# xxayt/MGSV

Measured on AMD Instinct MI355X. Metric: video-music pairs/s fwd+bwd at B=64 (full training step); sub-objects: retrieval sim-matrix GB/s, eval forward pairs/s, higher is better.
Workload: dtype bf16; 1 GPU; BASELINE.json configs[2]: B=64/GPU, T_v=30, T_a=512, D=512, train mode (dropout on), f32 master weights + Adam, f32 gradient accumulation; global_batch=64, launch=tape

## Files before the change

include/made_hip.h:

```cpp
#ifndef MADE_HIP_H
#define MADE_HIP_H

#include <stdint.h>

#ifdef __cplusplus
extern "C" {
#endif

#define MADE_ABI_VERSION 8

enum MadeDtype { MADE_F32 = 0, MADE_BF16 = 1 };

enum MadeAct {
    MADE_ACT_NONE = 0,
    MADE_ACT_RELU = 1,
    MADE_ACT_GELU = 2,
    MADE_ACT_QUICKGELU = 3,
    MADE_ACT_SIGMOID = 4
};

enum MadeGate {
    MADE_GATE_NONE = 0,
    MADE_GATE_RELU_OUT = 1,
    MADE_GATE_GELU_Z = 2,
// ... 20 lines not shown
MADE_HOST_DEVICE static inline uint32_t made_drop_threshold(float p) { return (uint32_t)((double)p * 16777216.0); }
MADE_HOST_DEVICE static inline uint32_t made_rng_key(uint64_t seed, uint32_t site, uint32_t idx_hi) {
    return made_rng_fmix32((uint32_t)seed ^ (site * 0x9E3779B9u) ^ ((uint32_t)(seed >> 32) * 0x85EBCA6Bu) ^ (idx_hi * 0xC2B2AE35u));
}
MADE_HOST_DEVICE static inline uint32_t made_rng_mix(uint64_t seed, uint32_t site, uint64_t idx) {
    return made_rng_fmix32((uint32_t)idx ^ made_rng_key(seed, site, (uint32_t)(idx >> 32)));
}
#if defined(__HIPCC__)
__device__ static inline uint64_t made_drop_seed(const MadeDropout& d) { return d.seed_device ? *d.seed_device : d.seed; }
#endif


enum MadeStatus {
    MADE_OK = 0,
    MADE_ERR_INVALID_ARG = -1,
    MADE_ERR_UNSUPPORTED = -2,
    MADE_ERR_HIP = -3
};

int         made_abi_version(void);
int         made_set_f32_products(int mode);
int         made_get_f32_products(void);
const char* made_last_error(void);
int         made_device_info(char* name, int name_len, int* cu_count, int* is_gfx950);

typedef struct MadeLinearSeg {
    int64_t col_begin;
    void*   out;
    int32_t out_dtype;
    int32_t transposed;
    int64_t ldo;
    int64_t rows_per_batch;
    int64_t out_batch_stride;
    int64_t out_z_stride;
    int32_t use_a2;
    int32_t _pad;
} MadeLinearSeg;

typedef struct MadeLinearArgs {
    const void*  A;  int32_t a_dtype; int32_t w_dtype;
    int64_t      lda;
    const void*  A2; int64_t lda2; int64_t a2_row_mod;
    int32_t      a2_replace;
    int32_t      drop_col_div;
    const float* a_row_mask;
    const void*  W;  int64_t ldw;
    const float* bias;
    int64_t      M, N, K;
    int64_t      batch, a_z_stride, w_z_stride;
    int32_t      act; int32_t r_dtype;
    const void*  R;  int64_t ldr; int64_t r_row_mod;
    const float* out_row_mask;
    const float* tile_skip_mask;
    int32_t      nseg; int32_t split_k;
    float*       split_ws;
    MadeLinearSeg seg[4];
    const void*  G;  int32_t g_dtype; int32_t gate;
    int64_t      ldg; float gate_scale; int32_t z_dtype;
    void*        Zout; int64_t ldz;
    MadeDropout  drop; int64_t drop_ld;
    const int32_t* row_index; const int32_t* n_rows;
    const float* bias_row_scale; int64_t bias_z_stride;
} MadeLinearArgs;

int made_linear(const MadeLinearArgs* args, void* stream);

enum MadeLinearVariant {
    MADE_LINEAR_GENERAL_F32 = 0,
    MADE_LINEAR_GENERAL_F32IN = 1,
    MADE_LINEAR_GENERAL_BF16 = 2,
    MADE_LINEAR_TINY = 3,
    MADE_LINEAR_SKINNY = 4,
    MADE_LINEAR_GLDS3 = 5,
    MADE_LINEAR_GLDS64 = 6,
    MADE_LINEAR_GLDS128 = 7,
    MADE_LINEAR_BIG256 = 8,
    MADE_LINEAR_TINY16 = 9,
    MADE_LINEAR_BIG128 = 10,
    MADE_LINEAR_GLDS64_F32 = 11,
    MADE_LINEAR_GLDS128_F32 = 12
};
int made_linear_variant(const MadeLinearArgs* args);

typedef struct MadeDecStageArgs {
    const void*  Zin; int64_t ldz;
    const float* ln_g; const float* ln_b;
    const float* ln2_g; const float* ln2_b; void* x2_out; int64_t ldx2;
    const void*  add; int64_t add_row_mod;
    void*        x_out; int64_t ldx;
    const void*  W; int64_t ldw; const float* bias;
    const void*  R; int64_t ldr;
    void*        out; int64_t ldo;
    int32_t      out_dtype; int32_t act; int32_t res_from_x; float eps;
    int64_t      M, N, K;
    int32_t      zin_dtype; int32_t drop_col_div;
    void*        a_out; int64_t lda_out;
    MadeDropout  drop; int64_t drop_ld;
} MadeDecStageArgs;
int made_dec_stage(const MadeDecStageArgs* args, void* stream);

typedef struct MadeDecStageBwdArgs {
    const void* xa; const float* gamma_a; int64_t ldxa;
    const void* xb; const float* gamma_b; int64_t ldxb;
    const void* dy; int64_t lddy;
    const void* add; int64_t ldadd;
    void* dx_out; int64_t lddx;
    void* a_out; int64_t lda_out;
    float *dgamma_a, *dbeta_a, *dgamma_b, *dbeta_b;
    MadeDropout drop_a; int64_t drop_a_ld;
    const void* W; int64_t ldw;
    const void* G; int64_t ldg; float gate_scale; float eps;
    MadeDropout drop_o; int64_t drop_o_ld; int32_t drop_o_col_div; int32_t _pad;
    const void* R; int64_t ldr;
    void* out; int64_t ldo;
    int64_t M, N, K;
} MadeDecStageBwdArgs;
int made_dec_stage_bwd(const MadeDecStageBwdArgs* args, void* stream);

typedef struct MadeFinishArgs {
    const float* ws; int64_t split_k, M, N;
    const float* bias; int32_t act; int32_t r_dtype;
    const void*  R; int64_t ldr; int64_t r_row_mod;
    void* out; int32_t out_dtype; int32_t _pad0; int64_t ldo;
    const float* ln1_g; const float* ln1_b; void* ln1_out; int32_t ln1_dtype; int32_t _pad1; int64_t ln1_ld;
    const float* ln2_g; const float* ln2_b; void* ln2_out; int32_t ln2_dtype; int32_t _pad2; int64_t ln2_ld;
    float eps; int32_t _pad3;
} MadeFinishArgs;

int made_splitk_finish(const MadeFinishArgs* args, void* stream);

typedef struct MadeAttnArgs {
    const void* Q; const void* K; const void* V; void* O;
    int32_t dtype; int32_t hd;
    int64_t B, H, Lq, Lk;
    int64_t q_bs, ldq, k_bs, ldk, v_bs, ldv, o_bs, ldo;
    const float* key_mask; const float* q_mask;
    float scale; int32_t _pad;
    const float* q_skip_mask;
    float*      lse;
    MadeDropout drop;
    const int32_t* batch_order;
    uint32_t* keep_bits;
    int64_t ld_bits;
} MadeAttnArgs;

int made_attention(const MadeAttnArgs* args, void* stream);

typedef struct MadeWideAttnArgs {
    const void* Q; const void* K; const void* Kadd; const void* V; void* O;
    const float* key_mask;
    int32_t dtype; int32_t o_dtype;
    int64_t B, NQ1, NQ2, L, D;
    int64_t q_bs, q_s1, q_s2, k_bs, ldk, kadd_bs, ldkadd, v_bs, ldv, o_bs, o_s1, o_s2;
    float scale; int32_t _pad;
    int64_t n_split;
    float*  part_o;
    float*  part_ml;
    MadeDropout drop;
    float*  sum_out;
    float*  lse_out;
} MadeWideAttnArgs;

int made_attention_wide(const MadeWideAttnArgs* args, void* stream);

typedef struct MadeWideAttnBwdArgs {
    const void *Q, *dO, *O, *K, *V;
// ... 219 lines not shown
typedef struct MadeGemmTNGroup {
    int32_t n_problems; float alpha;
    int64_t M, split_m;
    const int32_t* row_index; const int32_t* n_rows;
    MadeGemmTNProblem p[MADE_GEMM_TN_MAX_GROUP];
    int32_t tile_end[MADE_GEMM_TN_MAX_GROUP];
    int32_t tile_size; int32_t _pad;
    void* workspace; int64_t workspace_bytes;
} MadeGemmTNGroup;
int made_gemm_tn_grouped(const MadeGemmTNGroup* group, void* stream);
int64_t made_gemm_tn_grouped_workspace(const MadeGemmTNGroup* group);
int made_row_groups(const float* mask, int64_t M, float* out, void* stream);
int made_row_index(const float* mask, int64_t M, int32_t* row_index, int32_t* n_rows, void* stream);
int made_batch_order(const float* mask, int64_t B, int64_t T, int32_t* order, void* stream);

int made_layernorm_bwd(const void* x, int32_t x_dtype, int64_t ldx, int64_t x_rows_per_batch, int64_t x_batch_stride,
                       const float* gamma, const void* dy, int32_t dy_dtype, int64_t lddy,
                       const void* add, int32_t add_dtype, int64_t ld_add,
                       void* dx, int32_t dx_dtype, int64_t lddx,
                       void* dx_drop, int64_t lddxd, const MadeDropout* drop, int64_t drop_ld,
                       float* dgamma, float* dbeta, int64_t rows, int64_t D, float eps, const float* row_skip, void* stream);

int made_pool_bwd(const float* mean, const float* dvec, const float* mask,
                  const void* in1, int32_t in1_dtype, int64_t in1_bs, int64_t in1_ld,
                  const void* in2, int32_t in2_dtype, int64_t in2_bs, int64_t in2_ld,
                  void* out, int32_t out_dtype, int64_t out_bs, int64_t out_ld,
                  int64_t B, int64_t T, int64_t D, float eps, void* stream);

int made_l2norm_bwd(const void* x, int32_t x_dtype, int64_t ldx, const float* dy, int64_t lddy, int64_t dy_rows_per,
                    float* dx, int64_t lddx, int32_t accumulate, void* dx_alt, int32_t alt_dtype, int64_t lddxa,
                    int64_t rows, int64_t D, float eps, void* stream);

int made_clip_loss_bwd(const float* sims, int64_t ld, int64_t n, const float* logit_scale, float weight,
                       const float* upstream, float* lse_ws, float* dsims, float* dsims_t, int32_t accumulate,
                       float* d_logit_scale, const float* row_exclude, void* stream);

int made_xpool_tail_bwd(const void* y, int32_t y_dtype, int64_t ldy, const float* gamma, const float* beta,
                        const float* video, int64_t ld_video, const float* dsims, int64_t ld_dsims,
                        void* dy, int32_t dy_dtype, int64_t lddy, void* dy_drop, const MadeDropout* drop,
                        float* dgamma, float* dbeta, float* dvideo, int64_t ld_dvideo,
                        const float* dpool, int64_t ld_dpool, float dpool_scale,
                        int64_t Nm, int64_t Nv, int64_t D, float eps, void* stream);

int made_softmax_bwd(const float* S, int64_t ld_s, const float* dP, int64_t ld_dp, const float* mask, int64_t rows_per_mask,
                     const float* extra, float scale, const MadeDropout* drop,
                     void* Pd, void* dS, void* dSt, int32_t out_dtype, int64_t ldo, int64_t ldt,
                     int64_t out_batch_stride, int64_t t_batch_stride,
                     int64_t rows, int64_t rows_per_batch, int64_t L, void* stream);

int made_head_bias(void* x, int32_t x_dtype, int64_t ldx, const float* s, const float* bias, int64_t rows, int64_t H, int64_t hd,
                   void* stream);
int made_head_bias_bwd(const void* dy, int32_t dtype, int64_t ld, const float* s, const float* bias, float* dbias, float* ds,
                       int64_t rows, int64_t H, int64_t hd, void* stream);

int made_layernorm_bwd2(const void* xa, const float* gamma_a, int64_t ldxa, const void* xb, const float* gamma_b, int64_t ldxb,
                        const void* dy, int64_t lddy, const void* add, int64_t ld_add, void* dx, int64_t lddx,
                        void* dx_drop, int64_t lddxd, const MadeDropout* drop, int64_t drop_ld, int32_t dtype,
                        float* dgamma_a, float* dbeta_a, float* dgamma_b, float* dbeta_b, int64_t rows, int64_t D, float eps,
                        void* stream);

int made_gate_rows(const void* x, int32_t x_dtype, int64_t ldx, const void* G, int32_t g_dtype, int64_t ldg, int32_t gate,
                   float scale, const MadeDropout* drop, int64_t drop_ld, int64_t drop_col_div, void* out, int32_t out_dtype, int64_t ldo,
                   const float* row_skip, int64_t rows, int64_t cols, void* stream);
int made_add3(void* out, int32_t out_dtype, const void* a, int32_t a_dtype, const void* b, int32_t b_dtype,
              const void* c, int32_t c_dtype, int64_t n, int64_t b_mod, void* stream);
int made_colsum(const void* x, int32_t dtype, int64_t ld, int64_t rows, int64_t cols, float* out, void* stream);

int made_posbn_relu_fwd(const void* x, int32_t x_dtype, int64_t ldx, const float* weight, const float* bias,
                        float* running_mean, float* running_var, float momentum, float eps, int32_t batch_stats,
                        float* save_mean, float* save_rstd, void* y, int32_t y_dtype, int64_t ldy,
                        int64_t B, int64_t T, int64_t F, void* stream);
int made_posbn_relu_bwd(const void* x, int32_t x_dtype, int64_t ldx, const void* y, int32_t y_dtype, int64_t ldy,
                        const void* dy, int32_t dy_dtype, int64_t lddy, const float* weight, const float* save_mean,
                        const float* save_rstd, int32_t batch_stats, void* dx, int32_t dx_dtype, int64_t lddx,
                        float* dweight, float* dbias, int64_t B, int64_t T, int64_t F, void* stream);

int made_set_criterion_bwd(const float* pred_logits, const float* pred_spans, const float* targets,
                           const int64_t* pred_idx, const int64_t* tgt_idx, const int32_t* count,
                           const float* proj_queries, const float* vid_sum, const float* empty_weight,
                           int64_t n_layers, int64_t B, int64_t Q, int64_t G, int64_t Dc, int32_t fg_label,
                           float temperature, const float* weights, const float* upstream,
                           float* d_logits, float* d_spans, int64_t ld_out, int32_t through_sigmoid,
                           float* d_proj_queries, float* d_vid_sum, void* stream);

#define MADE_ADAM_MAX_GROUPS 4
#define MADE_ADAM_NORM_BLOCKS 1024
typedef struct MadeAdamGroup { int64_t begin, end; float lr; float max_norm; } MadeAdamGroup;
int made_adam_step(float* param, const float* grad, float* exp_avg, float* exp_avg_sq, int64_t n,
                   const MadeAdamGroup* groups, int32_t n_groups, float beta1, float beta2, float eps, int64_t step,
                   float grad_scale, float* norm_ws, void* stream);

typedef struct MadeAdamDeviceState { int64_t step; float lr[MADE_ADAM_MAX_GROUPS]; float bc1, bc2_sqrt; } MadeAdamDeviceState;
int made_adam_step_device(float* param, const float* grad, float* exp_avg, float* exp_avg_sq, int64_t n,
                          const MadeAdamGroup* groups, int32_t n_groups, float beta1, float beta2, float eps,
                          MadeAdamDeviceState* state_device, int32_t advance_state, float grad_scale, float* norm_ws, void* stream);

typedef struct MadeRepackDesc {
    const float* src; void* w; void* wt;
    int64_t rows, cols, wt_ld, tile_begin;
    int32_t dtype; int32_t _pad;
} MadeRepackDesc;
int made_repack(const MadeRepackDesc* descs_device, int32_t n_desc, int64_t total_tiles, void* stream);


int made_recall_ranks(const float* sims, int64_t ld, const int32_t* group_id, const int32_t* gt_group, int64_t Nv, int64_t Nm,
                      int64_t n_groups, int32_t* rank_out, int32_t* top1_out, void* stream);

int made_span_iou(const float* pred_logits, const float* pred_spans, const float* gt_moment, const float* m_duration,
                  int64_t N, int64_t Q, int32_t fg_label, float max_m_duration, float* iou_out, float* pred_out, void* stream);

int made_concat_cols(const float* a, int64_t cols_a, const float* c, int64_t cols_c, float* out, int64_t rows, void* stream);


int made_pooled_cosine(const float* anchor, int64_t lda, const void* pooled, int32_t pooled_dtype, float* out, int64_t sa, int64_t sp,
                       int64_t A, int64_t P, int64_t D, void* stream);
int made_scale_exp(const float* x, const float* logit_scale, float* out, int64_t n, void* stream);
int made_span_convert(const float* in, float* out, int64_t N, int32_t mode, void* stream);
int made_span_pairwise(const float* spans1, const float* spans2, float* iou, float* uni, float* giou, float* inter_over_2,
                       int64_t N, int64_t M, void* stream);
int made_span_iou_se(const float* pred_se, const float* gt_moment, const float* m_duration, int64_t N, float max_m_duration,
                     int32_t clamp_to_max, int32_t discounted, float* iou_out, void* stream);


int64_t made_topk_groups_ws_bytes(int64_t Nv, int64_t Nm, int64_t K);
int made_topk_groups(const float* sims, int64_t ld, const int32_t* group_id, int64_t Nv, int64_t Nm, int64_t n_groups,
                     int64_t K, int32_t* idx_out, float* score_out, void* ws, int64_t ws_bytes, void* stream);

int made_gather_pairs(const int32_t* vi, const int32_t* mi, int64_t P, int64_t Nv, int64_t Nm,
                      const void* v_tok, int64_t v_tok_stride, const float* v_mask, int64_t v_mask_stride,
                      const float* v_vec, int64_t v_vec_stride,
                      const void* m_tok, int64_t m_tok_stride, const float* m_mask, int64_t m_mask_stride,
                      const float* m_vec, int64_t m_vec_stride, int64_t Tv, int64_t Ta, int64_t D, int32_t dtype,
                      void* frame_out, int64_t frame_out_stride, void* seg_out, int64_t seg_out_stride,
                      float* fmask_out, float* smask_out, float* video_out, float* music_out, void* stream);


#define MADE_FRAMES_MAX (1 << 20)

typedef struct MadeFrameDesc {
    int64_t offset;
    int64_t coef;
    int32_t H, W;
    int32_t kh, kv;
} MadeFrameDesc;

int made_frames_preprocess(const uint8_t* frames, int64_t frames_bytes, const MadeFrameDesc* desc, int64_t n_frames,
                           const int32_t* coef, int64_t n_coef, void* patches, int32_t patch_dtype, int64_t ld_patch,
                           uint8_t* crop_out, void* stream);


#define MADE_AUDIO_TRACKS_MAX (1 << 16)
#define MADE_AUDIO_SEGS_MAX (1 << 20)
#define MADE_RESAMPLE_TILE 1024
#define MADE_RESAMPLE_SLAB 12288
#define MADE_AUDIO_ROWS 1024
#define MADE_AUDIO_MELS 128

typedef struct MadeResampleDesc {
    int64_t offset;
    int64_t n;
    int64_t taps;
    int32_t o, m;
    int32_t width;
    int32_t _pad;
} MadeResampleDesc;

// ... 18 lines not shown
```

mgsv_amd/_lib.py:

```python
from __future__ import annotations

import ctypes as C
import os

_HERE = os.path.dirname(os.path.abspath(__file__))


def variant_env(name: str, default: str = "") -> str:
    if os.environ.get("MADE_DEBUG_VARIANTS", "0") in ("", "0"):
        return default
    return os.environ.get(name, default)


LIB_PATH = os.environ.get("MADE_LIB_PATH") or os.path.join(_HERE, "libmade_hip.so")
ABI_VERSION = 8

F32, BF16 = 0, 1
ACT_NONE, ACT_RELU, ACT_GELU, ACT_QUICKGELU, ACT_SIGMOID = 0, 1, 2, 3, 4
GATE_NONE, GATE_RELU_OUT, GATE_GELU_Z, GATE_QUICKGELU_Z, GATE_SIGMOID_OUT = 0, 1, 2, 3, 4

vp, i64, i32, f32 = C.c_void_p, C.c_int64, C.c_int32, C.c_float

WIDE_PLAN_HEAD, WIDE_PLAN_SAMPLE, WIDE_PLAN_SLOT, WIDE_PLAN_SLOT_BITS = 4, 4, 16, 8

# ... 155 lines not shown

class MadeAdamDeviceState(C.Structure):
    _fields_ = [("step", i64), ("lr", f32 * 4), ("bc1", f32), ("bc2_sqrt", f32)]


class MadeRepackDesc(C.Structure):
    _fields_ = [("src", vp), ("w", vp), ("wt", vp), ("rows", i64), ("cols", i64), ("wt_ld", i64), ("tile_begin", i64),
                ("dtype", i32), ("_pad", i32)]


class MadeFrameDesc(C.Structure):
    _fields_ = [("offset", i64), ("coef", i64), ("H", i32), ("W", i32), ("kh", i32), ("kv", i32)]


class MadeResampleDesc(C.Structure):
    _fields_ = [("offset", i64), ("n", i64), ("taps", i64), ("o", i32), ("m", i32), ("width", i32), ("_pad", i32)]


class MadeAudioSegDesc(C.Structure):
    _fields_ = [("first", i64), ("count", i64)]


SIGNATURES = {
    "made_abi_version": (C.c_int, []),
    "made_set_f32_products": (C.c_int, [C.c_int]),
    "made_get_f32_products": (C.c_int, []),
    "made_last_error": (C.c_char_p, []),
    "made_device_info": (C.c_int, [C.c_char_p, C.c_int, C.POINTER(C.c_int), C.POINTER(C.c_int)]),
    "made_tape_begin": (C.c_int, []),
    "made_tape_end": (C.c_int, [C.POINTER(C.c_uint64)]),
    "made_tape_replay": (C.c_int, [C.c_uint64]),
    "made_tape_free": (C.c_int, [C.c_uint64]),
    "made_tape_interleave": (C.c_int, [C.c_uint64, i32]),
    "made_tape_count": (C.c_int, [C.c_uint64, C.POINTER(i64), C.POINTER(i64), C.POINTER(i64)]),
    "made_tape_replay_range": (C.c_int, [C.c_uint64, i64, i64]),
    "made_tape_op": (C.c_int, [C.c_uint64, i64, C.POINTER(i32), C.POINTER(C.c_uint64), C.POINTER(C.c_uint64), C.POINTER(C.c_uint32)]),
    "made_stream_wait": (C.c_int, [vp, vp]),
    "made_tape_event": (C.c_int, [i32, i32, vp]),
    "made_tape_callback": (C.c_int, [C.CFUNCTYPE(C.c_int, vp), vp]),
    "made_memset_async": (C.c_int, [vp, i32, i64, vp]),
    "made_copy_async": (C.c_int, [vp, vp, i64, vp]),
    "made_store_words": (C.c_int, [vp, vp, i32, vp]),
    "made_linear": (C.c_int, [C.POINTER(MadeLinearArgs), vp]),
    "made_splitk_finish": (C.c_int, [C.POINTER(MadeFinishArgs), vp]),
    "made_dec_stage": (C.c_int, [C.POINTER(MadeDecStageArgs), vp]),
    "made_dec_stage_bwd": (C.c_int, [C.POINTER(MadeDecStageBwdArgs), vp]),
    "made_attention": (C.c_int, [C.POINTER(MadeAttnArgs), vp]),
    "made_attention_wide": (C.c_int, [C.POINTER(MadeWideAttnArgs), vp]),
    "made_attention_wide_bwd": (C.c_int, [C.POINTER(MadeWideAttnBwdArgs), vp]),
    "made_wide_slice_plan": (C.c_int, [vp, i64, i64, i32, i32, vp, vp, i64, vp]),
    "made_attention_wide_planned": (C.c_int, [C.POINTER(MadeWideAttnArgs), vp, i32, vp]),
    "made_attention_wide_bwd_planned": (C.c_int, [C.POINTER(MadeWideAttnBwdArgs), vp, i32, vp]),
    "made_layernorm": (C.c_int, [vp, i32, i64, i64, i64, vp, vp, vp, i32, i64, i64, i64, f32, vp, vp]),
    "made_layernorm_add": (C.c_int, [vp, i32, i64, vp, vp, vp, i32, i64, vp, i32, i64, vp, i64, i64, i64, f32, vp, vp]),
    "made_cast_mask_rows": (C.c_int, [vp, i64, vp, vp, i32, i64, i64, i64, vp]),
    "made_pack_music_records": (C.c_int, [vp, i32, i64, vp, i64, vp, i64, vp, i32, i64, i64, i64, i64, i64, vp]),
    "made_masked_mean": (C.c_int, [vp, i32, i64, i64, vp, vp, i64, i64, i64, vp]),
    "made_l2norm_rows": (C.c_int, [vp, i32, i64, vp, vp, i32, i64, i64, i64, f32, vp]),
    "made_sine_pe": (C.c_int, [vp, vp, vp, i32, i64, i64, i64, vp]),
    "made_masked_softmax": (C.c_int, [vp, i64, vp, i64, vp, i32, i64, i64, i64, i64, i64, f32, vp]),
    "made_xpool_tail": (C.c_int, [vp, i32, i64, vp, vp, vp, i64, vp, vp, i64, i64, i64, i64, f32, vp]),
    "made_clip_loss": (C.c_int, [vp, i64, i64, vp, f32, i32, vp, vp, vp]),
    "made_hungarian_match": (C.c_int, [vp, vp, vp, i64, i64, i64, i64, i32, f32, f32, f32, vp, i32, vp, vp, vp, vp, vp]),
    "made_attention_bwd": (C.c_int, [C.POINTER(MadeAttnBwdArgs), vp]),
    "made_layernorm_bwd": (C.c_int, [vp, i32, i64, i64, i64, vp, vp, i32, i64, vp, i32, i64, vp, i32, i64, vp, i64,
                                     C.POINTER(MadeDropout), i64, vp, vp, i64, i64, f32, vp, vp]),
    "made_layernorm_bwd2": (C.c_int, [vp, vp, i64, vp, vp, i64, vp, i64, vp, i64, vp, i64, vp, i64, C.POINTER(MadeDropout), i64, i32,
                                      vp, vp, vp, vp, i64, i64, f32, vp]),
    "made_pool_bwd": (C.c_int, [vp, vp, vp, vp, i32, i64, i64, vp, i32, i64, i64, vp, i32, i64, i64, i64, i64, i64, f32, vp]),
    "made_l2norm_bwd": (C.c_int, [vp, i32, i64, vp, i64, i64, vp, i64, i32, vp, i32, i64, i64, i64, f32, vp]),
    "made_clip_loss_bwd": (C.c_int, [vp, i64, i64, vp, f32, vp, vp, vp, vp, i32, vp, vp, vp]),
    "made_xpool_tail_bwd": (C.c_int, [vp, i32, i64, vp, vp, vp, i64, vp, i64, vp, i32, i64, vp, C.POINTER(MadeDropout),
                                      vp, vp, vp, i64, vp, i64, f32, i64, i64, i64, f32, vp]),
    "made_softmax_bwd": (C.c_int, [vp, i64, vp, i64, vp, i64, vp, f32, C.POINTER(MadeDropout), vp, vp, vp, i32, i64, i64,
                                   i64, i64, i64, i64, i64, vp]),
    "made_head_bias": (C.c_int, [vp, i32, i64, vp, vp, i64, i64, i64, vp]),
    "made_head_bias_bwd": (C.c_int, [vp, i32, i64, vp, vp, vp, vp, i64, i64, i64, vp]),
    "made_add3": (C.c_int, [vp, i32, vp, i32, vp, i32, vp, i32, i64, i64, vp]),
    "made_colsum": (C.c_int, [vp, i32, i64, i64, i64, vp, vp]),
    "made_posbn_relu_fwd": (C.c_int, [vp, i32, i64, vp, vp, vp, vp, C.c_float, C.c_float, i32, vp, vp, vp, i32, i64, i64, i64, i64, vp]),
    "made_posbn_relu_bwd": (C.c_int, [vp, i32, i64, vp, i32, i64, vp, i32, i64, vp, vp, vp, i32, vp, i32, i64, vp, vp, i64, i64, i64, vp]),
    "made_set_criterion_bwd": (C.c_int, [vp, vp, vp, vp, vp, vp, vp, vp, vp, i64, i64, i64, i64, i64, i32, f32, vp, vp,
                                         vp, vp, i64, i32, vp, vp, vp]),
    "made_adam_step": (C.c_int, [vp, vp, vp, vp, i64, C.POINTER(MadeAdamGroup), i32, f32, f32, f32, i64, f32, vp, vp]),
    "made_adam_step_device": (C.c_int, [vp, vp, vp, vp, i64, C.POINTER(MadeAdamGroup), i32, f32, f32, f32, vp, i32, f32, vp, vp]),
    "made_repack": (C.c_int, [vp, i32, i64, vp]),
    "made_row_groups": (C.c_int, [vp, i64, vp, vp]),
    "made_row_index": (C.c_int, [vp, i64, vp, vp, vp]),
    "made_linear_variant": (C.c_int, [C.POINTER(MadeLinearArgs)]),
    "made_row_affine": (C.c_int, [vp, i32, i64, vp, vp, i64, i32, vp, i32, i64, i64, i64, vp]),
    "made_gate_rows": (C.c_int, [vp, i32, i64, vp, i32, i64, i32, f32, vp, i64, i64, vp, i32, i64, vp, i64, i64, vp]),
    "made_xpool_fused": (C.c_int, [C.POINTER(MadeXpoolFusedArgs), vp]),
    "made_xpool_attention": (C.c_int, [C.POINTER(MadeXpoolAttnArgs), vp]),
    "made_xpool_sims": (C.c_int, [C.POINTER(MadeXpoolSimsArgs), vp]),
    "made_xpool_sims_ws_bytes": (C.c_int64, [i64, i64, i64]),
    "made_xpool_inbatch": (C.c_int, [C.POINTER(MadeXpoolInbatchArgs), vp]),
    "made_xpool_inbatch_ws_bytes": (C.c_int64, [i64, i64]),
    "made_batch_order": (C.c_int, [vp, i64, i64, vp, vp]),
    "made_recall_ranks": (C.c_int, [vp, i64, vp, vp, i64, i64, i64, vp, vp, vp]),
    "made_span_iou": (C.c_int, [vp, vp, vp, vp, i64, i64, i32, f32, vp, vp, vp]),
    "made_gemm_tn": (C.c_int, [C.POINTER(MadeGemmTNArgs), vp]),
    "made_gemm_tn_grouped": (C.c_int, [C.POINTER(MadeGemmTNGroup), vp]),
    "made_gemm_tn_grouped_workspace": (i64, [C.POINTER(MadeGemmTNGroup)]),
    "made_concat_cols": (C.c_int, [vp, i64, vp, i64, vp, i64, vp]),
    "made_pooled_cosine": (C.c_int, [vp, i64, vp, i32, vp, i64, i64, i64, i64, i64, vp]),
    "made_scale_exp": (C.c_int, [vp, vp, vp, i64, vp]),
    "made_span_convert": (C.c_int, [vp, vp, i64, i32, vp]),
    "made_span_pairwise": (C.c_int, [vp, vp, vp, vp, vp, vp, i64, i64, vp]),
    "made_span_iou_se": (C.c_int, [vp, vp, vp, i64, f32, i32, i32, vp, vp]),
    "made_set_criterion": (C.c_int, [vp, vp, vp, vp, vp, vp, vp, vp, vp, i64, i64, i64, i64, i64, i32, f32, vp, vp, vp, vp]),
    "made_topk_groups_ws_bytes": (C.c_int64, [i64, i64, i64]),
    "made_topk_groups": (C.c_int, [vp, i64, vp, i64, i64, i64, i64, vp, vp, vp, i64, vp]),
    "made_gather_pairs": (C.c_int, [vp, vp, i64, i64, i64, vp, i64, vp, i64, vp, i64, vp, i64, vp, i64, vp, i64, i64, i64, i64, i32,
                                    vp, i64, vp, i64, vp, vp, vp, vp, vp]),
    "made_frames_preprocess": (C.c_int, [vp, i64, vp, i64, vp, i64, vp, i32, i64, vp, vp]),
    "made_audio_resample": (C.c_int, [vp, i64, vp, i64, vp, i64, vp, i64, vp]),
    "made_audio_fbank": (C.c_int, [vp, i64, vp, i64, vp, vp, vp, i32, vp, vp]),
    "made_ast_patches": (C.c_int, [vp, i64, vp, i32, i64, vp]),
}

_lib = None


class MadeError(RuntimeError):
    pass


def lib() -> C.CDLL:
    global _lib
    if _lib is None:
        if not os.path.isfile(LIB_PATH):
            raise MadeError(f"{LIB_PATH} not found: build the HIP library first (make -C mgsv_amd/csrc); "
                            "the MaDe hot path has no CPU fallback")
        l = C.CDLL(LIB_PATH)
        for name, (res, args) in SIGNATURES.items():
            fn = getattr(l, name)
            fn.restype = res
            fn.argtypes = args
        if l.made_abi_version() != ABI_VERSION:
            raise MadeError(f"ABI version mismatch: {LIB_PATH} is version {l.made_abi_version()}, this binding was written for {ABI_VERSION} "
                            "(rebuild: make -C mgsv_amd/csrc)")
        _lib = l
    return _lib


def check(status: int, what: str = "") -> None:
    if status != 0:
        msg = lib().made_last_error().decode("utf-8", "replace")
        raise MadeError(f"{what or 'libmade_hip'} failed (status {status}): {msg}")


def device_info():
    l = lib()
    name = C.create_string_buffer(64)
    cu, is950 = C.c_int(0), C.c_int(0)
    check(l.made_device_info(name, 64, C.byref(cu), C.byref(is950)), "made_device_info")
    return name.value.decode(), cu.value, bool(is950.value)
```

mgsv_amd/csrc/linear.hip:

```cpp
#include "common.h"

namespace {

constexpr int BM = 128, BN = 128;
constexpr int KB = 128;
constexpr int LDS_ROW = KB + 16;
constexpr int NTHREADS = 256;

template <typename TC> struct Frag;
template <> struct Frag<float>  { typedef f32x4  type; };
template <> struct Frag<bf16_t> { typedef bf16x8 type; };

template <typename TC>
__device__ __forceinline__ typename Frag<TC>::type zero_frag() {
    typename Frag<TC>::type z;
#pragma unroll
    for (int i = 0; i < elem_traits<TC>::per16; ++i) z[i] = (TC)0.f;
    return z;
}

template <typename TA, typename TC>
__device__ __forceinline__ typename Frag<TC>::type load_a_frag(const TA* __restrict__ p, const TA* __restrict__ p2) {
    constexpr int n = elem_traits<TC>::per16;
    float v[n];
// ... 1149 lines not shown
    for (int t = 0; t < 2; ++t)
#pragma unroll
        for (int e = 0; e < 16; ++e) acc[t][e] = 0.f;
    bf16x8 fa[2][T_CH][2], fw[2][T_CH];
    auto load = [&](int buf, int s0) __attribute__((always_inline)) {
#pragma unroll
        for (int i = 0; i < T_CH; ++i) {
            const int s = s0 + i < steps ? s0 + i : steps - 1;
            fw[buf][i] = *(const bf16x8*)(pw + s * 16);
            fa[buf][i][0] = *(const bf16x8*)(pa[0] + s * 16);
            fa[buf][i][1] = *(const bf16x8*)(pa[1] + s * 16);
        }
    };
    auto mul = [&](int buf, int s0) __attribute__((always_inline)) {
#pragma unroll
        for (int i = 0; i < T_CH; ++i) {
            if (s0 + i < steps) {
                acc[0] = __builtin_amdgcn_mfma_f32_32x32x16_bf16(fa[buf][i][0], fw[buf][i], acc[0], 0, 0, 0);
                acc[1] = __builtin_amdgcn_mfma_f32_32x32x16_bf16(fa[buf][i][1], fw[buf][i], acc[1], 0, 0, 0);
            }
        }
    };
    load(0, 0);
    for (int s0 = 0; s0 < steps; s0 += 2 * T_CH) {
        if (s0 + T_CH < steps) load(1, s0 + T_CH);
        mul(0, s0);
        if (s0 + 2 * T_CH < steps) load(0, s0 + 2 * T_CH);
        if (s0 + T_CH < steps) mul(1, s0 + T_CH);
    }

    float* mine = Ct + wave * (T_BM * T_CT_LD);
#pragma unroll
    for (int t = 0; t < 2; ++t)
#pragma unroll
        for (int e = 0; e < 16; ++e) mine[(t * 32 + acc_row(e, hh)) * T_CT_LD + r] = acc[t][e];
    __syncthreads();

    unsigned char* outp = (unsigned char*)seg.out;
    const int64_t out_z = z * seg.out_z_stride;
    const int rpb = (int)seg.rows_per_batch, rmod = (int)a.r_row_mod;
    const int colb = (int)seg.col_begin;
    const int cc = e_cc, row = e_row, n = e_n, nvalid = e_nvalid, ml = e_ml;
    if (nvalid <= 0 || ml >= Mv) return;
    float v[8];
#pragma unroll
    for (int j = 0; j < 8; ++j) v[j] = 0.f;
#pragma unroll
    for (int w = 0; w < 4; ++w) {
        const float* cp = Ct + w * (T_BM * T_CT_LD) + row * T_CT_LD + cc * 8;
        const f32x4 c0 = *(const f32x4*)cp, c1 = *(const f32x4*)(cp + 4);
        v[0] += c0[0]; v[1] += c0[1]; v[2] += c0[2]; v[3] += c0[3];
        v[4] += c1[0]; v[5] += c1[1]; v[6] += c1[2]; v[7] += c1[3];
    }
    const bool out_vec = (seg.ldo % 8 == 0) && (seg.out_batch_stride % 8 == 0) && (seg.out_z_stride % 8 == 0) &&
                         (((uintptr_t)outp & 15) == 0) && (colb % 8 == 0);
    const bool r_vec = a.R && (a.ldr % 8 == 0) && (((uintptr_t)a.R & 15) == 0);
    const int m = e_m;
    if (a.bias_row_scale) {
#pragma unroll
        for (int j = 0; j < 8; ++j) e_bv[j] *= e_bsc;
    }
    EpiPre pre;
    pre.has_r = e_rpref; pre.r = e_r; pre.has_g = e_gpref; pre.g = e_g; pre.has_om = true; pre.om = e_om;
    epilogue8<TRAIN>(a, m, n, nvalid, v, e_bv, rmod, r_vec, pre);
    int64_t orow;
    if (rpb > 0) {
        const int b = m / rpb, t = m - b * rpb;
        orow = (int64_t)b * seg.out_batch_stride + (int64_t)t * seg.ldo;
    } else {
        orow = (int64_t)m * seg.ldo;
    }
    store8(outp, seg.out_dtype, out_z + orow + (n - colb), v, nvalid, out_vec);
}

template <bool TRAIN>
__global__ __launch_bounds__(NTHREADS) void linear_tiny_kernel(const MadeLinearArgs a) {
    __shared__ __attribute__((aligned(16))) float Ct[4 * T_BM * T_CT_LD];
    linear_tiny_body<TRAIN>(a, blockIdx.x, blockIdx.z, Ct);
}

constexpr int U_BM = 16, U_BN = 16, U_CT_LD = U_BN + 4;

template <bool TRAIN, int SPW>
__global__ __launch_bounds__(NTHREADS) void linear_t16_kernel(const MadeLinearArgs a) {
    __shared__ __attribute__((aligned(16))) float Ct[4 * U_BM * U_CT_LD];
    const int tid = threadIdx.x;
    const int lane = tid & 63, wave = __builtin_amdgcn_readfirstlane(tid >> 6);
    const int r16 = lane & 15, kq = lane >> 4;
    const int M = (int)a.M, N = (int)a.N, K = (int)a.K;
    const int n_tiles = (N + U_BN - 1) / U_BN, m_tiles = (M + U_BM - 1) / U_BM;
    int tile_m, tile_n;
    {
        const int bx = blockIdx.x;
        if ((n_tiles & 7) == 0) { const int j = bx >> 3; tile_m = j % m_tiles; tile_n = (j / m_tiles) * 8 + (bx & 7); }
        else { tile_m = bx % m_tiles; tile_n = bx / m_tiles; }
    }
    const int m0 = tile_m * U_BM, n0 = tile_n * U_BN;
    const int64_t z = blockIdx.z;
    int Mv = M;
    if (a.n_rows) { const int nv = *a.n_rows; Mv = nv < M ? nv : M; }
    if (m0 >= Mv) return;
    int si = 0;
#pragma unroll
    for (int s = 1; s < 4; ++s)
        if (s < a.nseg && n0 >= a.seg[s].col_begin) si = s;
    const MadeLinearSeg seg = a.seg[si];
    const bool repl = seg.use_a2 && a.A2 && a.a2_replace;
    const bf16_t* Abase = (repl ? (const bf16_t*)a.A2 : (const bf16_t*)a.A) + z * a.a_z_stride;
    const int64_t lda = repl ? a.lda2 : a.lda;
    const int steps = K / 32;
    int gm = m0 + r16; gm = gm < Mv ? gm : Mv - 1;
    if (a.row_index) gm = a.row_index[gm];
    int gn = n0 + r16; gn = gn < N ? gn : N - 1;
    const bf16_t* pa = Abase + (int64_t)gm * lda + kq * 8;
    const bf16_t* pw = (const bf16_t*)a.W + z * a.w_z_stride + (int64_t)gn * a.ldw + kq * 8;
    bf16x8 fa[SPW], fw[SPW];
#pragma unroll
    for (int i = 0; i < SPW; ++i) {
        int s = wave + 4 * i; s = s < steps ? s : steps - 1;
        fw[i] = *(const bf16x8*)(pw + s * 32);
        fa[i] = *(const bf16x8*)(pa + s * 32);
    }
    const int e_cc = tid & 1, e_row = (tid >> 1) & 15;
    const int e_n = n0 + e_cc * 8;
    int e_nvalid = N - e_n; e_nvalid = e_nvalid > 8 ? 8 : e_nvalid;
    const int e_ml = m0 + e_row;
    int e_m = e_ml < Mv ? e_ml : Mv - 1;
    if (a.row_index) e_m = a.row_index[e_m];
    float e_bv[8];
    load_bias8(a.bias_row_scale ? a.bias + z * a.bias_z_stride : a.bias, e_n, N, e_bv);
    float e_bsc = 1.f;
    if (a.bias_row_scale) e_bsc = a.bias_row_scale[(int64_t)e_m * a.batch + z];
    const int e_rmod = (int)a.r_row_mod;
    const bool e_rpref = a.R && a.r_dtype == MADE_BF16 && (a.ldr % 8 == 0) && (((uintptr_t)a.R & 15) == 0) && e_nvalid == 8;
    const bool e_gpref = TRAIN && a.gate != MADE_GATE_NONE && a.g_dtype == MADE_BF16 && (a.ldg % 8 == 0) && (((uintptr_t)a.G & 15) == 0) && e_nvalid == 8;
    bf16x8 e_r = {}, e_g = {};
    if (e_rpref) e_r = *(const bf16x8*)((const bf16_t*)a.R + (int64_t)(e_rmod > 0 ? e_m % e_rmod : e_m) * a.ldr + e_n);
    if constexpr (TRAIN) { if (e_gpref) e_g = *(const bf16x8*)((const bf16_t*)a.G + (int64_t)e_m * a.ldg + e_n); }
    float e_om = 1.f;
    if (a.out_row_mask) e_om = a.out_row_mask[e_m];
    uint64_t e_seed = 0;
    if constexpr (TRAIN) { if (a.drop.p > 0.f) e_seed = made_drop_seed(a.drop); }

    f32x4 acc;
    acc[0] = acc[1] = acc[2] = acc[3] = 0.f;
#pragma unroll
    for (int i = 0; i < SPW; ++i)
        if (wave + 4 * i < steps) acc = __builtin_amdgcn_mfma_f32_16x16x32_bf16(fa[i], fw[i], acc, 0, 0, 0);
    float* mine = Ct + wave * (U_BM * U_CT_LD);
#pragma unroll
    for (int e = 0; e < 4; ++e) mine[(kq * 4 + e) * U_CT_LD + r16] = acc[e];
    __syncthreads();
    if (tid >= 32) return;
    const int n = e_n, nvalid = e_nvalid;
    if (nvalid <= 0 || e_ml >= Mv) return;
    float v[8];
#pragma unroll
    for (int j = 0; j < 8; ++j) v[j] = 0.f;
#pragma unroll
    for (int w = 0; w < 4; ++w) {
        const float* cp = Ct + w * (U_BM * U_CT_LD) + e_row * U_CT_LD + e_cc * 8;
        const f32x4 c0 = *(const f32x4*)cp, c1 = *(const f32x4*)(cp + 4);
        v[0] += c0[0]; v[1] += c0[1]; v[2] += c0[2]; v[3] += c0[3];
        v[4] += c1[0]; v[5] += c1[1]; v[6] += c1[2]; v[7] += c1[3];
    }
    unsigned char* outp = (unsigned char*)seg.out;
    const int64_t out_z = z * seg.out_z_stride;
    const int rpb = (int)seg.rows_per_batch, rmod = (int)a.r_row_mod;
    const int colb = (int)seg.col_begin;
    const bool out_vec = (seg.ldo % 8 == 0) && (seg.out_batch_stride % 8 == 0) && (seg.out_z_stride % 8 == 0) &&
                         (((uintptr_t)outp & 15) == 0) && (colb % 8 == 0);
    const bool r_vec = a.R && (a.ldr % 8 == 0) && (((uintptr_t)a.R & 15) == 0);
    const int m = e_m;
    if (a.bias_row_scale) {
#pragma unroll
        for (int j = 0; j < 8; ++j) e_bv[j] *= e_bsc;
    }
    EpiPre pre;
    pre.has_r = e_rpref; pre.r = e_r; pre.has_g = e_gpref; pre.g = e_g; pre.has_om = true; pre.om = e_om;
    pre.has_seed = TRAIN && a.drop.p > 0.f; pre.seed = e_seed;
    epilogue8<TRAIN>(a, m, n, nvalid, v, e_bv, rmod, r_vec, pre);
    int64_t orow;
    if (rpb > 0) {
        const int b = m / rpb, t = m - b * rpb;
        orow = (int64_t)b * seg.out_batch_stride + (int64_t)t * seg.ldo;
    } else {
        orow = (int64_t)m * seg.ldo;
    }
    store8(outp, seg.out_dtype, out_z + orow + (n - colb), v, nvalid, out_vec);
}

template <bool TRAIN>
static void launch_t16(const MadeLinearArgs& a, hipStream_t st) {
    const int steps = (int)(a.K / 32), spw = (steps + 3) / 4;
    dim3 g((unsigned)(((a.M + U_BM - 1) / U_BM) * ((a.N + U_BN - 1) / U_BN)), 1, (unsigned)a.batch), block(NTHREADS);
    if (spw <= 1) hipLaunchKernelGGL((linear_t16_kernel<TRAIN, 1>), g, block, 0, st, a);
    else if (spw <= 2) hipLaunchKernelGGL((linear_t16_kernel<TRAIN, 2>), g, block, 0, st, a);
    else if (spw <= 4) hipLaunchKernelGGL((linear_t16_kernel<TRAIN, 4>), g, block, 0, st, a);
    else hipLaunchKernelGGL((linear_t16_kernel<TRAIN, 8>), g, block, 0, st, a);
}

}


static int tile_pref() {
    const char* e = made_variant_env("MADE_LINEAR_TILE");
    return e ? atoi(e) : 0;
}

static int64_t tiny_max() {
    const char* e = made_variant_env("MADE_TINY_MAX");
    return e ? (int64_t)atoll(e) : 1024;
}

static int64_t f32_glds_min() {
    const char* e = made_variant_env("MADE_LINEAR_F32_GLDS_MIN");
    return e ? (int64_t)atoll(e) : 1;
}

static int64_t big_train_min() {
    const char* e = made_variant_env("MADE_LINEAR_BIG_TRAIN");
    return e ? (int64_t)atoll(e) : 0;
}

static int64_t t16_max() {
    static const int64_t v = [] { const char* e = made_variant_env("MADE_T16_MAX"); return e ? (int64_t)atoll(e) : (int64_t)4096; }();
    return v;
}

static bool big_fast_epilogue(const MadeLinearArgs& a) {
    auto al = [](const void* p, int64_t ld, int dt) { return (((uintptr_t)p & 15) == 0) && ld % (dt == MADE_BF16 ? 8 : 4) == 0; };
    bool ok = (a.act == MADE_ACT_NONE || a.act == MADE_ACT_RELU) && a.N % 8 == 0 && (a.gate == MADE_GATE_NONE || a.gate == MADE_GATE_RELU_OUT);
    if (a.gate != MADE_GATE_NONE) ok = ok && al(a.G, a.ldg, a.g_dtype);
    if (a.Zout) ok = ok && al(a.Zout, a.ldz, a.z_dtype);
    if (a.R) ok = ok && al(a.R, a.ldr, a.r_dtype);
    if (a.drop.p > 0.f) ok = ok && a.drop_col_div <= 1;
    for (int s = 0; s < a.nseg; ++s)
        ok = ok && a.seg[s].rows_per_batch == 0 && a.seg[s].col_begin % 8 == 0 && al(a.seg[s].out, a.seg[s].ldo, a.seg[s].out_dtype);
    return ok;
}

static int pick_variant(const MadeLinearArgs& a) {
    if (a.w_dtype != MADE_BF16) {
        bool fast = a.a_dtype == MADE_F32 && a.K % 32 == 0 && a.a_row_mask == nullptr && a.split_k <= 1 && (a.A2 == nullptr || a.a2_replace) &&
                    ((uintptr_t)a.A % 16 == 0) && ((uintptr_t)a.W % 16 == 0) && (a.lda % 4 == 0) && (a.ldw % 4 == 0) && a.bias_row_scale == nullptr &&
                    made_variant_env("MADE_LINEAR_F32_GLDS_OFF") == nullptr;
        for (int s = 0; s < a.nseg; ++s) fast = fast && !a.seg[s].transposed;
        if (a.A2 && a.a2_replace) fast = fast && (a.a2_row_mod == 0) && (a.lda2 % 4 == 0) && ((uintptr_t)a.A2 % 16 == 0);
        if (a.batch > 1) fast = fast && (a.a_z_stride % 4 == 0) && (a.w_z_stride % 4 == 0);
        const int64_t tiles = ((a.M + BM - 1) / BM) * ((a.N + BN - 1) / BN);
        const int64_t tiles64 = ((a.M + 63) / 64) * ((a.N + BN - 1) / BN);
        if (fast && tiles64 * a.batch >= f32_glds_min()) {
            const int64_t live = a.row_index ? (tiles * a.batch * 9) / 16 : tiles * a.batch;
            return live > 1280 ? MADE_LINEAR_GLDS128_F32 : MADE_LINEAR_GLDS64_F32;
        }
        return MADE_LINEAR_GENERAL_F32;
    }
    bool fast = a.a_dtype == MADE_BF16 && a.K % 64 == 0 && a.a_row_mask == nullptr && a.split_k <= 1 &&
                (a.A2 == nullptr || a.a2_replace) && ((uintptr_t)a.A % 16 == 0) && (a.lda % 8 == 0);
    for (int s = 0; s < a.nseg; ++s) fast = fast && !a.seg[s].transposed;
    if (a.A2 && a.a2_replace) fast = fast && (a.a2_row_mod == 0) && (a.lda2 % 8 == 0);
    if (!fast) return a.a_dtype == MADE_F32 ? MADE_LINEAR_GENERAL_F32IN : MADE_LINEAR_GENERAL_BF16;
    const int64_t tiles = ((a.M + BM - 1) / BM) * ((a.N + BN - 1) / BN);
    const int64_t tiles64 = ((a.M + S_BM - 1) / S_BM) * ((a.N + S_BN - 1) / S_BN);
    const int64_t tiles32 = ((a.M + T_BM - 1) / T_BM) * ((a.N + T_BN - 1) / T_BN);
    if (a.M <= 64 && a.K >= 128 && a.K <= 1024 && a.K % 32 == 0 && a.tile_skip_mask == nullptr && tile_pref() != 1 && tile_pref() != 32 &&
        ((a.M + 15) / 16) * ((a.N + 15) / 16) * a.batch <= t16_max())
        return MADE_LINEAR_TINY16;
    if (tiles32 * a.batch <= tiny_max() && a.K <= 1024 && a.tile_skip_mask == nullptr && tile_pref() != 1) return MADE_LINEAR_TINY;
    if (tiles64 * a.batch <= 256 && a.tile_skip_mask == nullptr) return MADE_LINEAR_SKINNY;
    if (tiles * a.batch <= 256) return MADE_LINEAR_GLDS3;
    {
        const bool train_like = a.gate != MADE_GATE_NONE || a.Zout != nullptr || a.drop.p > 0.f;
        bool big_ok = a.batch == 1 && a.tile_skip_mask == nullptr && a.N <= BIG_NMAX && a.ldw % 8 == 0 && (!train_like || big_fast_epilogue(a));
        for (int s = 0; s < a.nseg; ++s) big_ok = big_ok && (a.seg[s].col_begin % BIG_BN == 0) && a.seg[s].out_z_stride == 0;
        if (big_ok) {
            if (tile_pref() == 512) return MADE_LINEAR_BIG256;
            if (tile_pref() == 256) return MADE_LINEAR_BIG128;
            const int64_t tiles256 = ((a.M + 255) / 256) * ((a.N + BIG_BN - 1) / BIG_BN);
            if (tile_pref() == 0 && !a.row_index && tiles256 >= 2 * 256) return MADE_LINEAR_BIG256;
            const int64_t tiles128 = ((a.M + 127) / 128) * ((a.N + BIG_BN - 1) / BIG_BN);
            const int64_t live128 = a.row_index ? (tiles128 * 9) / 16 : tiles128;
// ... 76 lines not shown
    const bool train = a.gate != MADE_GATE_NONE || a.Zout != nullptr || a.drop.p > 0.f;
    switch (pick_variant(a)) {
        case MADE_LINEAR_TINY16:
            if (train) launch_t16<true>(a, st); else launch_t16<false>(a, st);
            break;
        case MADE_LINEAR_TINY: {
            dim3 g32((unsigned)(((a.M + T_BM - 1) / T_BM) * ((a.N + T_BN - 1) / T_BN)), 1, (unsigned)a.batch);
            if (train) hipLaunchKernelGGL((linear_tiny_kernel<true>), g32, block, 0, st, a);
            else hipLaunchKernelGGL((linear_tiny_kernel<false>), g32, block, 0, st, a);
            break;
        }
        case MADE_LINEAR_SKINNY: {
            dim3 g64((unsigned)(((a.M + S_BM - 1) / S_BM) * ((a.N + S_BN - 1) / S_BN)), 1, (unsigned)a.batch);
            if (train) hipLaunchKernelGGL((linear_skinny_kernel<true>), g64, block, 0, st, a);
            else hipLaunchKernelGGL((linear_skinny_kernel<false>), g64, block, 0, st, a);
            break;
        }
        case MADE_LINEAR_GLDS3:
            if (train) hipLaunchKernelGGL((linear_glds_kernel<3, true, 128>), grid, block, 0, st, a);
            else hipLaunchKernelGGL((linear_glds_kernel<3, false, 128>), grid, block, 0, st, a);
            break;
        case MADE_LINEAR_GLDS64: {
            dim3 g((unsigned)(((a.M + 63) / 64) * ((a.N + BN - 1) / BN)), 1, (unsigned)a.batch);
            if (train) hipLaunchKernelGGL((linear_glds_kernel<1, true, 64>), g, block, 0, st, a);
            else hipLaunchKernelGGL((linear_glds_kernel<1, false, 64>), g, block, 0, st, a);
            break;
        }
        case MADE_LINEAR_GLDS128:
            if (train) hipLaunchKernelGGL((linear_glds_kernel<1, true, 128>), grid, block, 0, st, a);
            else hipLaunchKernelGGL((linear_glds_kernel<1, false, 128>), grid, block, 0, st, a);
            break;
        case MADE_LINEAR_GLDS64_F32: {
            dim3 g((unsigned)(((a.M + 63) / 64) * ((a.N + BN - 1) / BN)), 1, (unsigned)a.batch);
            if (train) { if (g_made_f32_products) hipLaunchKernelGGL((linear_glds_kernel<1, true, 64, float, true>), g, block, 0, st, a); else hipLaunchKernelGGL((linear_glds_kernel<1, true, 64, float>), g, block, 0, st, a); }
            else { if (g_made_f32_products) hipLaunchKernelGGL((linear_glds_kernel<1, false, 64, float, true>), g, block, 0, st, a); else hipLaunchKernelGGL((linear_glds_kernel<1, false, 64, float>), g, block, 0, st, a); }
            break;
        }
        case MADE_LINEAR_GLDS128_F32:
            if (train) { if (g_made_f32_products) hipLaunchKernelGGL((linear_glds_kernel<1, true, 128, float, true>), grid, block, 0, st, a); else hipLaunchKernelGGL((linear_glds_kernel<1, true, 128, float>), grid, block, 0, st, a); }
            else { if (g_made_f32_products) hipLaunchKernelGGL((linear_glds_kernel<1, false, 128, float, true>), grid, block, 0, st, a); else hipLaunchKernelGGL((linear_glds_kernel<1, false, 128, float>), grid, block, 0, st, a); }
            break;
        case MADE_LINEAR_BIG256:
        case MADE_LINEAR_BIG128: {
            const bool b256 = pick_variant(a) == MADE_LINEAR_BIG256;
            const int bmb = b256 ? 256 : 128;
            const int ldsb = 2 * (bmb + BIG_BN) * KB + BIG_NMAX * 4;
            static const int n_cu = [] { int dev = 0, n = 0; (void)hipGetDevice(&dev); (void)hipDeviceGetAttribute(&n, hipDeviceAttributeMultiprocessorCount, dev); return n > 8 ? n : 256; }();
            static const bool once = [] {
                constexpr int l256 = 2 * (256 + BIG_BN) * KB + BIG_NMAX * 4, l128 = 2 * (128 + BIG_BN) * KB + BIG_NMAX * 4;
                bool ok = true;
                ok = ok && hipFuncSetAttribute((const void*)linear_big_kernel<256, false, false>, hipFuncAttributeMaxDynamicSharedMemorySize, l256) == hipSuccess;
                ok = ok && hipFuncSetAttribute((const void*)linear_big_kernel<256, false, true>, hipFuncAttributeMaxDynamicSharedMemorySize, l256) == hipSuccess;
                ok = ok && hipFuncSetAttribute((const void*)linear_big_kernel<128, false, false>, hipFuncAttributeMaxDynamicSharedMemorySize, l128) == hipSuccess;
                ok = ok && hipFuncSetAttribute((const void*)linear_big_kernel<128, false, true>, hipFuncAttributeMaxDynamicSharedMemorySize, l128) == hipSuccess;
                ok = ok && hipFuncSetAttribute((const void*)linear_big_kernel<256, true, true>, hipFuncAttributeMaxDynamicSharedMemorySize, l256) == hipSuccess;
                ok = ok && hipFuncSetAttribute((const void*)linear_big_kernel<128, true, true>, hipFuncAttributeMaxDynamicSharedMemorySize, l128) == hipSuccess;
                return ok;
            }();
            (void)once;
            const int64_t nt = ((a.M + bmb - 1) / bmb) * ((a.N + BIG_BN - 1) / BIG_BN);
            int64_t g = (n_cu / 8) * 8;
            if (nt < g) g = ((nt + 7) / 8) * 8;
            dim3 gb((unsigned)g), bb(BIG_THREADS);
            const bool fastep = big_fast_epilogue(a);
            const bool lite = fastep && (train || a.R != nullptr || a.out_row_mask != nullptr);
            if (b256) {
                if (lite) hipLaunchKernelGGL((linear_big_kernel<256, true, true>), gb, bb, ldsb, st, a);
                else if (fastep) hipLaunchKernelGGL((linear_big_kernel<256, false, true>), gb, bb, ldsb, st, a);
                else hipLaunchKernelGGL((linear_big_kernel<256, false, false>), gb, bb, ldsb, st, a);
            } else {
                if (lite) hipLaunchKernelGGL((linear_big_kernel<128, true, true>), gb, bb, ldsb, st, a);
                else if (fastep) hipLaunchKernelGGL((linear_big_kernel<128, false, true>), gb, bb, ldsb, st, a);
                else hipLaunchKernelGGL((linear_big_kernel<128, false, false>), gb, bb, ldsb, st, a);
            }
            break;
        }
        case MADE_LINEAR_GENERAL_F32IN: hipLaunchKernelGGL((linear_kernel<float, bf16_t>), grid, block, 0, st, a); break;
        case MADE_LINEAR_GENERAL_BF16: hipLaunchKernelGGL((linear_kernel<bf16_t, bf16_t>), grid, block, 0, st, a); break;
        default: if (g_made_f32_products) hipLaunchKernelGGL((linear_kernel<float, float, true>), grid, block, 0, st, a); else hipLaunchKernelGGL((linear_kernel<float, float>), grid, block, 0, st, a); break;
    }
    return made_check_launch("made_linear");
}

extern "C" int made_linear_variant(const MadeLinearArgs* args) {
    return args ? pick_variant(*args) : -1;
}
```

mgsv_amd/csrc/matcher.hip:

```cpp
#include "common.h"
#pragma clang fp contract(off)

namespace {

constexpr int MAXN = 64;

__device__ __forceinline__ float giou_se(float s1, float e1, float s2, float e2) {
    float a1 = __fsub_rn(e1, s1), a2 = __fsub_rn(e2, s2);
    float inter = fmaxf(__fsub_rn(fminf(e1, e2), fmaxf(s1, s2)), 0.f);
    float uni = __fsub_rn(__fadd_rn(a1, a2), inter);
    float iou = __fdiv_rn(inter, uni);
    float enc = fmaxf(__fsub_rn(fmaxf(e1, e2), fminf(s1, s2)), 0.f);
    return __fsub_rn(iou, __fdiv_rn(__fsub_rn(enc, uni), enc));
}

__device__ __forceinline__ void cw_to_se(float c, float w, float& s, float& e) {
    float hw = __fmul_rn(0.5f, w);
    s = __fsub_rn(c, hw);
    e = __fadd_rn(c, hw);
}

__global__ __launch_bounds__(64) void hungarian_kernel(const float* logits, const float* spans, const float* targets,
                                                       int B, int Q, int G, int fg, float w_span, float w_giou, float w_class,
                                                       float* cost_ws, int cost_is_input, int64_t* out_pred, int64_t* out_tgt,
// ... 162 lines not shown
                d += __shfl_xor(d, 1);
                d += __shfl_xor(d, 2);
                if (part == 0) lgt[i] = d / temperature;
            }
        }
        __syncthreads();
        float span_sum = 0.f, giou_sum = 0.f, correct = 0.f, npairs = 0.f;
        for (int i = tid; i < B * width; i += CRIT_THREADS) {
            int b = i / width, slot = i % width;
            int s = l * B + b;
            if (slot < count[s]) {
                int q = (int)pred_idx[(int64_t)s * width + slot];
                int g = kth_kept(targets + (int64_t)b * G * 2, G, (int)tgt_idx[(int64_t)s * width + slot]);
                float pc = sp[(b * Q + q) * 2], pw = sp[(b * Q + q) * 2 + 1];
                float tc = targets[((int64_t)b * G + g) * 2], tw = targets[((int64_t)b * G + g) * 2 + 1];
                span_sum += fabsf(pc - tc) + fabsf(pw - tw);
                float ps, pe, ts, te;
                cw_to_se(pc, pw, ps, pe);
                cw_to_se(tc, tw, ts, te);
                giou_sum += 1.f - giou_se(ps, pe, ts, te);
                float l0 = lg[(b * Q + q) * 2], l1 = lg[(b * Q + q) * 2 + 1];
                int top = l1 > l0 ? 1 : 0;
                correct += (top == fg) ? 1.f : 0.f;
                npairs += 1.f;
                matched[b * Q + q] = 1;
            }
        }
        span_sum = block_sum(span_sum, red);
        giou_sum = block_sum(giou_sum, red);
        correct = block_sum(correct, red);
        npairs = block_sum(npairs, red);
        float label_sum = 0.f;
        for (int i = tid; i < B * Q; i += CRIT_THREADS) {
            int cls = matched[i] ? fg : bg;
            float l0 = lg[i * 2], l1 = lg[i * 2 + 1];
            float mx = fmaxf(l0, l1);
            float lse = mx + logf(expf(l0 - mx) + expf(l1 - mx));
            label_sum += empty_w[cls] * (lse - (cls == 0 ? l0 : l1));
        }
        label_sum = block_sum(label_sum, red);
        float contr = 0.f;
        if (proj_q && vid_sum) {
            float csum = 0.f;
            for (int b = tid; b < B; b += CRIT_THREADS) {
                float mx = -INFINITY, pos = 0.f, npos = 0.f;
                for (int q = 0; q < Q; ++q) {
                    float z = lgt[b * Q + q];
                    mx = fmaxf(mx, z);
                    if (matched[b * Q + q]) { pos += z; npos += 1.f; }
                }
                float se = 0.f;
                for (int q = 0; q < Q; ++q) se += expf(lgt[b * Q + q] - mx);
                csum += -pos / npos + (mx + logf(se));
            }
            contr = block_sum(csum, red) / (float)B;
        }
        if (tid == 0) {
            float ls = span_sum / (2.f * npairs);
            float lgi = giou_sum / npairs;
            float ll = label_sum / (float)(B * Q);
            float ce = 100.f - correct * (100.f / npairs);
            float* o = losses + l * 5;
            o[0] = ls; o[1] = lgi; o[2] = ll; o[3] = ce; o[4] = contr;
        }
    }
}

__global__ void criterion_total_kernel(const float* losses, const float* weights, int n_layers, float* total) {
    if (threadIdx.x != 0) return;
    float t = 0.f;
    for (int l = 0; l < n_layers; ++l) {
        const float* o = losses + l * 5;
        t += weights[0] * o[0] + weights[1] * o[1] + weights[2] * o[2] + weights[4] * o[4];
    }
    total[0] = t;
}

__global__ __launch_bounds__(CRIT_THREADS) void criterion_bwd_kernel(const float* logits, const float* spans, const float* targets,
                                                                     const int64_t* pred_idx, const int64_t* tgt_idx, const int32_t* count,
                                                                     const float* proj_q, const float* vid_sum, const float* empty_w,
                                                                     int B, int Q, int G, int Dc, int fg, float temperature,
                                                                     const float* weights, const float* upstream,
                                                                     float* dlogits, float* dspans, int ldo, int through_sigmoid,
                                                                     float* dproj_q, float* dvid_sum) {
    __shared__ unsigned char matched[CRIT_MAX_BQ];
    __shared__ float lgt[CRIT_MAX_BQ];
    __shared__ float red[4];
    const int tid = threadIdx.x, lane = tid & 63, wave = tid >> 6;
    const int width = Q < G ? Q : G;
    const int bg = 1 - fg;
    const int l = blockIdx.x;
    const int slice = blockIdx.y, nslice = gridDim.y;
    const float up = upstream ? upstream[0] : 1.f;
    const float* lg = logits + (int64_t)l * B * Q * 2;
    const float* sp = spans + (int64_t)l * B * Q * 2;
    float* dlg = dlogits + (int64_t)l * B * Q * ldo;
    float* dsp = dspans + (int64_t)l * B * Q * ldo;
    for (int i = tid; i < B * Q; i += CRIT_THREADS) {
        matched[i] = 0;
        if (slice == 0) { dsp[ldo * i] = 0.f; dsp[ldo * i + 1] = 0.f; }
    }
    __syncthreads();
    float npairs = 0.f;
    for (int i = tid; i < B * width; i += CRIT_THREADS) {
        int b = i / width, slot = i % width;
        if (slot < count[l * B + b]) npairs += 1.f;
    }
    npairs = block_sum(npairs, red);
    for (int i = tid; i < B * width; i += CRIT_THREADS) {
        int b = i / width, slot = i % width;
        int s = l * B + b;
        if (slot < count[s]) {
            int q = (int)pred_idx[(int64_t)s * width + slot];
            matched[b * Q + q] = 1;
            if (slice != 0) continue;
            int g = kth_kept(targets + (int64_t)b * G * 2, G, (int)tgt_idx[(int64_t)s * width + slot]);
            float pc = sp[(b * Q + q) * 2], pw = sp[(b * Q + q) * 2 + 1];
            float tc = targets[((int64_t)b * G + g) * 2], tw = targets[((int64_t)b * G + g) * 2 + 1];
            const float wl1 = up * weights[0] / (2.f * npairs);
            float dc = wl1 * (pc > tc ? 1.f : (pc < tc ? -1.f : 0.f));
            float dw = wl1 * (pw > tw ? 1.f : (pw < tw ? -1.f : 0.f));
            float ps, pe, ts, te;
            cw_to_se(pc, pw, ps, pe);
            cw_to_se(tc, tw, ts, te);
            const float mn_e = fminf(pe, te), mx_s = fmaxf(ps, ts);
            const float inter = fmaxf(mn_e - mx_s, 0.f);
            const float uni = (pe - ps) + (te - ts) - inter;
            const float enc = fmaxf(fmaxf(pe, te) - fminf(ps, ts), 0.f);
            const float pos_i = (mn_e - mx_s) > 0.f ? 1.f : 0.f;
            const float di_pe = pos_i * (pe <= te ? 1.f : 0.f), di_ps = -pos_i * (ps >= ts ? 1.f : 0.f);
            const float du_pe = 1.f - di_pe, du_ps = -1.f - di_ps;
            const float pos_e = enc > 0.f ? 1.f : 0.f;
            const float de_pe = pos_e * (pe >= te ? 1.f : 0.f), de_ps = -pos_e * (ps <= ts ? 1.f : 0.f);
            const float dg_pe = (di_pe * uni - inter * du_pe) / (uni * uni) + (du_pe * enc - uni * de_pe) / (enc * enc);
            const float dg_ps = (di_ps * uni - inter * du_ps) / (uni * uni) + (du_ps * enc - uni * de_ps) / (enc * enc);
            const float wg = -up * weights[1] / npairs;
            dc += wg * (dg_pe + dg_ps);
            dw += wg * 0.5f * (dg_pe - dg_ps);
            if (through_sigmoid) { dc *= pc * (1.f - pc); dw *= pw * (1.f - pw); }
            dsp[(b * Q + q) * ldo] = dc;
            dsp[(b * Q + q) * ldo + 1] = dw;
        }
    }
    __syncthreads();
    for (int i = tid; i < B * Q && slice == 0; i += CRIT_THREADS) {
        int cls = matched[i] ? fg : bg;
        float l0 = lg[i * 2], l1 = lg[i * 2 + 1];
        float mx = fmaxf(l0, l1);
        float e0 = expf(l0 - mx), e1 = expf(l1 - mx);
        float p0 = e0 / (e0 + e1), p1 = e1 / (e0 + e1);
        const float w = up * weights[2] * empty_w[cls] / (float)(B * Q);
        dlg[i * ldo] = w * (p0 - (cls == 0 ? 1.f : 0.f));
        dlg[i * ldo + 1] = w * (p1 - (cls == 1 ? 1.f : 0.f));
    }
    if (proj_q && vid_sum && dproj_q && dvid_sum) {
        const int nrow = ((B - slice + nslice - 1) / nslice) * Q;
        for (int j = wave; j < nrow; j += CRIT_THREADS / 64) {
            const int b = slice + (j / Q) * nslice, i = b * Q + j % Q;
            const float* pq = proj_q + ((int64_t)l * B * Q + i) * Dc;
            const float* vs = vid_sum + (int64_t)b * Dc;
            float d = 0.f;
            for (int k = lane; k < Dc; k += 64) d += pq[k] * vs[k];
            d = wave_sum(d);
            if (lane == 0) lgt[i] = d / temperature;
        }
        __syncthreads();
        const float wc = up * weights[4] / ((float)B * temperature);
        for (int j = wave; j < nrow; j += CRIT_THREADS / 64) {
            const int b = slice + (j / Q) * nslice, i = b * Q + j % Q;
            float mx = -INFINITY, npos = 0.f;
            for (int q = 0; q < Q; ++q) { mx = fmaxf(mx, lgt[b * Q + q]); npos += matched[b * Q + q] ? 1.f : 0.f; }
            float se = 0.f;
            for (int q = 0; q < Q; ++q) se += expf(lgt[b * Q + q] - mx);
            const float dl = wc * (expf(lgt[i] - mx) / se - (matched[i] ? 1.f / npos : 0.f));
            const float* pq = proj_q + ((int64_t)l * B * Q + i) * Dc;
            const float* vs = vid_sum + (int64_t)b * Dc;
            float* dpq = dproj_q + ((int64_t)l * B * Q + i) * Dc;
            for (int k = lane; k < Dc; k += 64) {
                dpq[k] = dl * vs[k];
                unsafeAtomicAdd(dvid_sum + (int64_t)b * Dc + k, dl * pq[k]);
            }
        }
    }
}

}

extern "C" int made_hungarian_match(const float* pred_logits, const float* pred_spans, const float* targets,
                                    int64_t NS, int64_t B, int64_t Q, int64_t G, int32_t fg_label,
                                    float w_span, float w_giou, float w_class,
                                    float* cost_ws, int32_t cost_is_input, int64_t* out_pred_idx, int64_t* out_tgt_idx,
                                    int32_t* out_count, int32_t* status, void* stream) {
    MADE_REQUIRE(pred_logits && pred_spans && targets && cost_ws && out_pred_idx && out_tgt_idx && out_count && status,
                 "made_hungarian_match: null pointer");
    MADE_REQUIRE(NS >= 0 && B > 0 && NS % B == 0, "made_hungarian_match: NS=%lld must be a multiple of B=%lld", (long long)NS, (long long)B);
    MADE_REQUIRE(fg_label == 0 || fg_label == 1, "made_hungarian_match: fg_label must be 0 or 1");
    MADE_UNSUPPORTED(Q >= 1 && G >= 1 && Q <= MAXN && G <= MAXN, "made_hungarian_match: Q=%lld, G=%lld must be in [1,%d]",
                     (long long)Q, (long long)G, MAXN);
    if (NS == 0) return MADE_OK;
    hipLaunchKernelGGL(hungarian_kernel, dim3((unsigned)NS), dim3(64), 0, (hipStream_t)stream, pred_logits, pred_spans, targets,
                       (int)B, (int)Q, (int)G, (int)fg_label, w_span, w_giou, w_class, cost_ws, (int)cost_is_input, out_pred_idx, out_tgt_idx,
                       out_count, status);
    return made_check_launch("made_hungarian_match");
}

extern "C" int made_set_criterion(const float* pred_logits, const float* pred_spans, const float* targets,
                                  const int64_t* pred_idx, const int64_t* tgt_idx, const int32_t* count,
                                  const float* proj_queries, const float* vid_sum, const float* empty_weight,
                                  int64_t n_layers, int64_t B, int64_t Q, int64_t G, int64_t Dc, int32_t fg_label,
                                  float temperature, const float* weights, float* losses, float* total, void* stream) {
    MADE_REQUIRE(pred_logits && pred_spans && targets && pred_idx && tgt_idx && count && empty_weight && weights && losses,
                 "made_set_criterion: null pointer");
    MADE_REQUIRE(n_layers >= 1 && B >= 1 && Q >= 1 && G >= 1, "made_set_criterion: bad dims");
    MADE_UNSUPPORTED(n_layers <= 65535 && B * Q <= CRIT_MAX_BQ, "made_set_criterion: B*Q=%lld exceeds %d", (long long)(B * Q), CRIT_MAX_BQ);
    hipLaunchKernelGGL(criterion_kernel, dim3((unsigned)n_layers), dim3(CRIT_THREADS), 0, (hipStream_t)stream, pred_logits, pred_spans, targets,
                       pred_idx, tgt_idx, count, proj_queries, vid_sum, empty_weight, (int)n_layers, (int)B, (int)Q, (int)G,
                       (int)Dc, (int)fg_label, temperature, weights, losses, total);
    int rc = made_check_launch("made_set_criterion");
    if (rc != MADE_OK || total == nullptr) return rc;
    hipLaunchKernelGGL(criterion_total_kernel, dim3(1), dim3(64), 0, (hipStream_t)stream, losses, weights, (int)n_layers, total);
    return made_check_launch("made_set_criterion(total)");
}

extern "C" int made_set_criterion_bwd(const float* pred_logits, const float* pred_spans, const float* targets,
                                      const int64_t* pred_idx, const int64_t* tgt_idx, const int32_t* count,
                                      const float* proj_queries, const float* vid_sum, const float* empty_weight,
                                      int64_t n_layers, int64_t B, int64_t Q, int64_t G, int64_t Dc, int32_t fg_label,
                                      float temperature, const float* weights, const float* upstream,
                                      float* d_logits, float* d_spans, int64_t ld_out, int32_t through_sigmoid,
                                      float* d_proj_queries, float* d_vid_sum, void* stream) {
    MADE_REQUIRE(pred_logits && pred_spans && targets && pred_idx && tgt_idx && count && empty_weight && weights && d_logits && d_spans,
                 "made_set_criterion_bwd: null pointer");
    MADE_REQUIRE(n_layers >= 1 && B >= 1 && Q >= 1 && G >= 1, "made_set_criterion_bwd: bad dims");
    MADE_UNSUPPORTED(n_layers <= 65535 && B * Q <= CRIT_MAX_BQ, "made_set_criterion_bwd: B*Q=%lld exceeds %d", (long long)(B * Q), CRIT_MAX_BQ);
    const unsigned nslice = (proj_queries && vid_sum && d_proj_queries && d_vid_sum) ? (unsigned)(B < 16 ? B : 16) : 1u;
    hipLaunchKernelGGL(criterion_bwd_kernel, dim3((unsigned)n_layers, nslice), dim3(CRIT_THREADS), 0, (hipStream_t)stream, pred_logits, pred_spans,
                       targets, pred_idx, tgt_idx, count, proj_queries, vid_sum, empty_weight, (int)B, (int)Q, (int)G, (int)Dc,
                       (int)fg_label, temperature, weights, upstream, d_logits, d_spans, (int)(ld_out > 0 ? ld_out : 2), (int)through_sigmoid,
                       d_proj_queries, d_vid_sum);
    return made_check_launch("made_set_criterion_bwd");
}
```

mgsv_amd/ops.py:

```python
from __future__ import annotations

import ctypes as C
import math
from dataclasses import dataclass
from typing import NamedTuple, Optional, Sequence

import torch

from . import _lib, tape as _tape
from ._lib import (ACT_GELU, ACT_NONE, ACT_QUICKGELU, ACT_RELU, ACT_SIGMOID, BF16, F32,
                   MadeAttnArgs, MadeDecStageArgs, MadeFinishArgs, MadeLinearArgs, MadeLinearSeg, MadeWideAttnArgs, check, lib)

Tensor = torch.Tensor


def dt_of(t: Tensor) -> int:
    if t.dtype == torch.float32:
        return F32
    if t.dtype == torch.bfloat16:
        return BF16
    raise TypeError(f"unsupported dtype {t.dtype}")


def torch_dtype(code: int):
# ... 39 lines not shown
    def __init__(self):
        self.records = []

    def __enter__(self):
        global _timer
        self._prev, _timer = _timer, self
        return self

    def __exit__(self, *exc):
        global _timer
        _timer = self._prev

    def summary(self):
        torch.cuda.synchronize()
        out = {}
        frac_cache = {}
        for kind, s, e, flops, nbytes, desc in self.records:
            d = out.setdefault(kind, dict(launches=0, ms=0.0, flops=0.0, bytes=0.0, flops_nominal=0.0))
            d["launches"] += 1
            d["ms"] += s.elapsed_time(e)
            frac = 1.0
            if isinstance(desc, tuple) and desc[0] == "rows":
                frac = min(1.0, (math.ceil(int(desc[1].item()) / 128) * 128) / max(desc[2], 1))
            elif isinstance(desc, tuple) and desc[0] == "attn":
                key = ("attn", desc[1].data_ptr() if desc[1] is not None else 0, desc[2].data_ptr() if desc[2] is not None else 0)
                if key not in frac_cache:
                    fk = (desc[1] != 0).float().mean(dim=1) if desc[1] is not None else 1.0
                    fq = (desc[2] != 0).float().mean(dim=1) if desc[2] is not None else 1.0
                    f = fk * fq
                    frac_cache[key] = float(f.mean().item()) if isinstance(f, torch.Tensor) else 1.0
                frac = frac_cache[key]
            elif isinstance(desc, tuple) and desc[0] == "frac":
                frac = float(desc[1])
            elif isinstance(desc, tuple):
                _, mask, tile = desc
                key = (mask.data_ptr(), mask.numel(), tile)
                if key not in frac_cache:
                    n = mask.numel()
                    pad = (-n) % tile
                    m = torch.nn.functional.pad(mask.reshape(-1) != 0, (0, pad)).view(-1, tile)
                    frac_cache[key] = float(m.any(dim=1).float().mean().item())
                frac = frac_cache[key]
            d["flops"] += flops * frac
            d["bytes"] += nbytes * frac
            d["flops_nominal"] += flops
        return out


_timer: Optional[KernelTimer] = None


def _timed(kind: str, flops: float, nbytes: float, launch, desc: str = ""):
    if _timer is None:
        return launch()
    s, e = torch.cuda.Event(enable_timing=True), torch.cuda.Event(enable_timing=True)
    s.record()
    r = launch()
    e.record()
    _timer.records.append((kind, s, e, flops, nbytes, desc))
    return r


@dataclass
class Seg:
    out: Tensor
    col_begin: int = 0
    ldo: Optional[int] = None
    transposed: bool = False
    rows_per_batch: int = 0
    out_batch_stride: int = 0
    out_z_stride: int = 0
    use_a2: bool = False


LINEAR_VARIANTS = {0: "linear_f32", 1: "linear_f32in_bf16", 2: "linear_kernel<bf16,bf16>", 3: "linear_tiny_kernel", 4: "linear_skinny_kernel",
                   5: "linear_glds_kernel<3,.,128>", 6: "linear_glds_kernel<1,.,64>", 7: "linear_glds_kernel<1,.,128>",
                   8: "linear_big_kernel<256>", 9: "linear_t16_kernel", 10: "linear_big_kernel<128>",
                   11: "linear_glds_f32<64>", 12: "linear_glds_f32<128>"}


LINEAR_LOG = None


def linear(A: Tensor, W: Tensor, bias: Optional[Tensor] = None, *, out: Optional[Tensor] = None,
           segs: Optional[Sequence[Seg]] = None, A2: Optional[Tensor] = None, a2_row_mod: int = 0,
           a2_replace: bool = False, a_row_mask: Optional[Tensor] = None, act: int = ACT_NONE, R: Optional[Tensor] = None,
           r_row_mod: int = 0, out_row_mask: Optional[Tensor] = None, out_dtype: Optional[torch.dtype] = None,
           tile_skip_mask: Optional[Tensor] = None, batch: int = 1, a_z_stride: int = 0, w_z_stride: int = 0, M: Optional[int] = None,
           N: Optional[int] = None, K: Optional[int] = None, gate: int = 0, G: Optional[Tensor] = None, gate_scale: float = 1.0,
           Zout: Optional[Tensor] = None, drop=None, drop_ld: Optional[int] = None, rows=None, drop_col_div: int = 1,
           bias_row_scale: Optional[Tensor] = None, bias_z_stride: int = 0) -> Tensor:
    assert A.dim() == 2 and W.dim() == 2 and A.stride(1) == 1 and W.stride(1) == 1
    M = A.shape[0] if M is None else M
    K = A.shape[1] if K is None else K
    N = W.shape[0] if N is None else N
    a = MadeLinearArgs()
    a.A, a.a_dtype, a.w_dtype, a.lda = _p(A), dt_of(A), dt_of(W), A.stride(0)
    if A2 is not None:
        assert A2.dim() == 2 and A2.stride(1) == 1 and A2.dtype == A.dtype
        a.A2, a.lda2, a.a2_row_mod = _p(A2), A2.stride(0), a2_row_mod
        a.a2_replace = 1 if a2_replace else 0
    a.a_row_mask = _p(_f32(a_row_mask, "a_row_mask"))
    a.W, a.ldw = _p(W), W.stride(0)
    a.bias = _p(_f32(bias, "bias"))
    a.M, a.N, a.K = M, N, K
    a.batch, a.a_z_stride, a.w_z_stride = batch, a_z_stride, w_z_stride
    a.act = act
    if R is not None:
        assert R.dim() == 2 and R.stride(1) == 1
        a.R, a.r_dtype, a.ldr, a.r_row_mod = _p(R), dt_of(R), R.stride(0), r_row_mod
    a.out_row_mask = _p(_f32(out_row_mask, "out_row_mask"))
    a.tile_skip_mask = _p(_f32(tile_skip_mask, "tile_skip_mask"))
    if gate:
        assert G is not None and G.dim() == 2 and G.stride(1) == 1
        a.G, a.g_dtype, a.gate, a.ldg, a.gate_scale = _p(G), dt_of(G), gate, G.stride(0), float(gate_scale)
    if Zout is not None:
        assert Zout.dim() == 2 and Zout.stride(1) == 1
        a.Zout, a.z_dtype, a.ldz = _p(Zout), dt_of(Zout), Zout.stride(0)
    if drop is not None and drop[2] > 0.0:
        set_drop(a.drop, drop)
        a.drop_ld = N if drop_ld is None else drop_ld
        a.drop_col_div = int(drop_col_div)
    if rows is not None:
        a.row_index, a.n_rows = _p(rows[0]), _p(rows[1])
    if bias_row_scale is not None:
        assert tuple(bias_row_scale.shape) == (M, batch)
        a.bias_row_scale, a.bias_z_stride = _p(_f32(bias_row_scale, "bias_row_scale")), bias_z_stride
    if segs is None:
        if out is None:
            out = torch.empty((M, N) if batch == 1 else (batch, M, N), device=A.device,
                              dtype=out_dtype or W.dtype)
        segs = [Seg(out=out, out_z_stride=(out.stride(0) if (batch > 1 and out.dim() == 3) else 0))]
    a.nseg = len(segs)
    for i, s in enumerate(segs):
        sg = a.seg[i]
        sg.col_begin, sg.out, sg.out_dtype = s.col_begin, _p(s.out), dt_of(s.out)
        sg.transposed = 1 if s.transposed else 0
        sg.ldo = s.ldo if s.ldo is not None else s.out.stride(-2)
        sg.rows_per_batch, sg.out_batch_stride, sg.out_z_stride = s.rows_per_batch, s.out_batch_stride, s.out_z_stride
        sg.use_a2 = 1 if s.use_a2 else 0
    esz = 4 if a.w_dtype == F32 else 2
    kind = "linear_" + ("f32" if a.w_dtype == F32 else ("bf16" if a.a_dtype == BF16 else "f32in_bf16"))
    if _timer is not None and kind == "linear_bf16":
        kind = LINEAR_VARIANTS[lib().made_linear_variant(C.byref(a))]
    elif _timer is not None and kind == "linear_f32" and lib().made_linear_variant(C.byref(a)) >= 11:
        kind = LINEAR_VARIANTS[lib().made_linear_variant(C.byref(a))]
    flops = 2.0 * M * N * K * batch
    nbytes = batch * (M * K * (4 if a.a_dtype == F32 else 2) + N * K * esz + M * N * esz)
    desc = f"M={M} N={N} K={K} z={batch} nseg={len(segs)} a2={int(A2 is not None)} R={int(R is not None)} act={act} tr={int(any(s_.transposed for s_ in segs))}"
    if LINEAR_LOG is not None:
        LINEAR_LOG.append((LINEAR_VARIANTS.get(lib().made_linear_variant(C.byref(a)), "?") if kind in ("linear_bf16", "linear_f32") else kind, M, N, K, batch,
                           f"nseg={len(segs)} a2={int(A2 is not None)}/{int(bool(a2_replace))} R={None if R is None else str(R.dtype)[6:]}/{r_row_mod} act={act} gate={gate} "
                           f"G={None if G is None else str(G.dtype)[6:]} Z={None if Zout is None else str(Zout.dtype)[6:]} "
                           f"drop={0 if drop is None else drop[2]}/{drop_col_div} rows={int(rows is not None)} orm={int(out_row_mask is not None)} "
                           f"arm={int(a_row_mask is not None)} out={str(segs[0].out.dtype)[6:]} rpb={segs[0].rows_per_batch} tr={int(any(s_.transposed for s_ in segs))}"))
    _timed(kind, flops, nbytes, lambda: check(lib().made_linear(C.byref(a), _stream()), "made_linear"),
           ("rows", rows[1], M) if rows is not None else ((desc, tile_skip_mask, 128) if tile_skip_mask is not None else desc))
    return segs[0].out


def row_index(mask: Tensor, out=None):
    m = mask.reshape(-1)
    M = m.numel()
    if out is not None:
        idx, n = out
        assert idx.dtype == torch.int32 and idx.numel() >= M and n.dtype == torch.int32
    else:
        idx = torch.empty(M, device=m.device, dtype=torch.int32)
        n = torch.empty(1, device=m.device, dtype=torch.int32)
    check(lib().made_row_index(_p(_f32(m, "mask")), M, _p(idx), _p(n), _stream()), "made_row_index")
    return idx, n


def batch_order(mask: Tensor, out: Optional[Tensor] = None) -> Tensor:
    assert mask.dim() == 2
    B, T = mask.shape
    if out is None:
        out = torch.empty(B, device=mask.device, dtype=torch.int32)
    assert out.dtype == torch.int32 and out.numel() == B
    check(lib().made_batch_order(_p(_f32(mask.contiguous(), "mask")), B, T, _p(out), _stream()), "made_batch_order")
    return out


def linear_splitk(A: Tensor, W: Tensor, bias: Optional[Tensor], ws: Tensor, split_k: int, *, A2: Optional[Tensor] = None,
                  a2_row_mod: int = 0, act: int = ACT_NONE, R: Optional[Tensor] = None, r_row_mod: int = 0,
                  out: Optional[Tensor] = None, ln1=None, ln1_out: Optional[Tensor] = None, ln2=None,
                  ln2_out: Optional[Tensor] = None, eps: float = 1e-5) -> None:
    assert A.dim() == 2 and W.dim() == 2 and A.stride(1) == 1 and W.stride(1) == 1
    M, K = A.shape
    N = W.shape[0]
    assert ws.dtype == torch.float32 and ws.is_contiguous() and ws.numel() >= split_k * M * N
    a = MadeLinearArgs()
    a.A, a.a_dtype, a.w_dtype, a.lda = _p(A), dt_of(A), dt_of(W), A.stride(0)
    use_a2 = A2 is not None
    if use_a2:
        a.A2, a.lda2, a.a2_row_mod = _p(A2), A2.stride(0), a2_row_mod
    a.W, a.ldw = _p(W), W.stride(0)
    a.M, a.N, a.K = M, N, K
    a.batch = 1
    a.nseg, a.split_k, a.split_ws = 1, max(split_k, 2), _p(ws)
    sg = a.seg[0]
    sg.col_begin, sg.out, sg.out_dtype, sg.ldo, sg.use_a2 = 0, _p(ws), F32, N, 1 if use_a2 else 0
    esz = 4 if a.w_dtype == F32 else 2
    _timed("linear_splitk_f32" if a.w_dtype == F32 else "linear_kernel<bf16,bf16>", 2.0 * M * N * K, M * K * esz + N * K * esz + M * N * 4 * a.split_k,
           lambda: check(lib().made_linear(C.byref(a), _stream()), "made_linear(split_k)"), f"M={M} N={N} K={K} split={a.split_k}")
    splitk_finish(ws, a.split_k, M, N, bias, act=act, R=R, r_row_mod=r_row_mod, out=out, ln1=ln1, ln1_out=ln1_out, ln2=ln2, ln2_out=ln2_out,
                  eps=eps)


def splitk_finish(ws: Tensor, split_k: int, M: int, N: int, bias: Optional[Tensor], *, act: int = ACT_NONE, R: Optional[Tensor] = None,
                  r_row_mod: int = 0, out: Optional[Tensor] = None, ln1=None, ln1_out: Optional[Tensor] = None, ln2=None,
                  ln2_out: Optional[Tensor] = None, eps: float = 1e-5) -> None:
    assert ws.dtype == torch.float32 and ws.is_contiguous() and ws.numel() >= split_k * M * N
    f = MadeFinishArgs()
    f.ws, f.split_k, f.M, f.N = _p(ws), split_k, M, N
    f.bias, f.act = _p(_f32(bias, "bias")), act
    if R is not None:
        assert R.dim() == 2 and R.stride(1) == 1
        f.R, f.r_dtype, f.ldr, f.r_row_mod = _p(R), dt_of(R), R.stride(0), r_row_mod
    if out is not None:
        f.out, f.out_dtype, f.ldo = _p(out), dt_of(out), out.stride(0)
    if ln1 is not None:
        f.ln1_g, f.ln1_b = _p(_f32(ln1[0], "ln1.g")), _p(_f32(ln1[1], "ln1.b"))
        if ln1_out is not None:
            f.ln1_out, f.ln1_dtype, f.ln1_ld = _p(ln1_out), dt_of(ln1_out), ln1_out.stride(0)
    if ln2 is not None:
        f.ln2_g, f.ln2_b = _p(_f32(ln2[0], "ln2.g")), _p(_f32(ln2[1], "ln2.b"))
        f.ln2_out, f.ln2_dtype, f.ln2_ld = _p(ln2_out), dt_of(ln2_out), ln2_out.stride(0)
    f.eps = eps
    check(lib().made_splitk_finish(C.byref(f), _stream()), "made_splitk_finish")


def dec_stage(Zin: Tensor, W: Tensor, bias: Optional[Tensor], out: Tensor, *, ln=None, ln2=None, x2_out: Optional[Tensor] = None,
              add: Optional[Tensor] = None, x_out: Optional[Tensor] = None, R: Optional[Tensor] = None, res_from_x: bool = False,
              act: int = ACT_NONE, eps: float = 1e-5, a_out: Optional[Tensor] = None, drop=None, drop_ld: Optional[int] = None,
              drop_col_div: int = 1) -> Tensor:
    assert Zin.dim() == 2 and W.dim() == 2 and out.dim() == 2 and W.dtype == torch.bfloat16
    assert Zin.stride(1) == 1 and W.stride(1) == 1 and out.stride(1) == 1
    M, K = Zin.shape
    N = W.shape[0]
    assert W.shape[1] == K and tuple(out.shape) == (M, N)
# ... 557 lines not shown
```

mgsv_amd/ops_train.py:

```python
from __future__ import annotations

import ctypes as C
from typing import Optional, Tuple

import torch

from . import _lib
from ._lib import BF16, F32, MadeAttnBwdArgs, MadeDropout, MadeGemmTNArgs, MadeGemmTNGroup, check, lib
from .ops import _f32, _p, _stream, _timed, dt_of, set_drop

Tensor = torch.Tensor
Pair = Tuple[int, int]


_TN_SLAB_US = 1.3


def _tn_splits(tiles: int, nslab: int, gathered: bool, cap: int) -> int:
    if _lib.variant_env("MADE_TN_SPLIT_MODEL", "1") == "0":
        sp = max(8, (512 // max(tiles, 1)) // 8 * 8) if cap == 64 and tiles < 64 else max(1, 2048 // max(tiles, 1))
        while (nslab + sp - 1) // sp > 64:
            sp += 8
        return min(sp, max(1, nslab))
    live = max(1, (nslab * 9) // 16 if gathered else nslab)
# ... 304 lines not shown
    a.key_mask, a.lse, a.ssum, a.extra = _p(_f32(key_mask, "key_mask")), _p(_f32(lse, "lse")), _p(_f32(ssum, "ssum")), _p(_f32(extra, "extra"))
    if dattc is not None:
        assert dattc.dim() == 2 and dattc.dtype == torch.bfloat16 and dattc.stride(1) == 1 and vbias is not None
        a.dattc, a.ld_dattc, a.vbias, a.hd = _p(dattc), dattc.stride(0), _p(_f32(vbias, "vbias")), hd
    a.Pd, a.dS, a.p_bs, a.ld_p = _p(Pd), _p(dS), Pd.stride(0), Pd.stride(1)
    a.dQ, a.dq_bs, a.ld_dq = _p(dQ), dQ.stride(0), dQ.stride(1)
    a.B, a.NQ, a.L, a.D = B, NQ, L, D
    a.q_bs, a.ld_q, a.do_bs, a.ld_do, a.o_bs, a.ld_o = Q.stride(0), Q.stride(1), dO.stride(0), dO.stride(1), O.stride(0), O.stride(1)
    a.k_bs, a.ldk, a.v_bs, a.ldv = K.stride(0), K.stride(1), V.stride(0), V.stride(1)
    a.scale = float(scale)
    if plan is not None:
        assert key_mask is not None and (plan.B, plan.L) == (B, L) and n_split >= plan.max_slices, "the plan is not this call's"
    if n_split > 1 or plan is not None:
        assert part_dq is not None and part_dq.dtype == torch.float32 and part_dq.numel() >= B * n_split * NQ * D
        a.n_split, a.part_dq = n_split, _p(part_dq)
    if drop is not None and drop[2] > 0.0:
        set_drop(a.drop, drop)
    _timed("made_attention_wide_bwd", 6.0 * B * NQ * L * D, 2.0 * B * (2 * L * D + 4 * NQ * D + 2 * NQ * L),
                (lambda: check(lib().made_attention_wide_bwd(C.byref(a), _stream()), "made_attention_wide_bwd")) if plan is None else
                (lambda: check(lib().made_attention_wide_bwd_planned(C.byref(a), _p(plan.words), plan.n_slots, _stream()), "made_attention_wide_bwd_planned")),
                f"B={B} NQ={NQ} L={L} D={D}" + (" planned" if plan is not None else ""))
    return dQ


def head_bias(x: Tensor, s: Tensor, bias: Tensor, H: int) -> None:
    rows, D = x.shape
    check(lib().made_head_bias(_p(x), dt_of(x), x.stride(0), _p(_f32(s, "s")), _p(bias), rows, H, D // H, _stream()), "made_head_bias")


def head_bias_bwd(dy: Tensor, s: Tensor, bias: Tensor, dbias: Tensor, ds: Tensor, H: int) -> None:
    rows, D = dy.shape
    check(lib().made_head_bias_bwd(_p(dy), dt_of(dy), dy.stride(0), _p(_f32(s, "s")), _p(bias), _p(dbias), _p(ds), rows, H, D // H,
                                   _stream()), "made_head_bias_bwd")


def add3(out: Tensor, a: Tensor, b: Optional[Tensor] = None, c: Optional[Tensor] = None, b_mod: int = 0) -> Tensor:
    for t in (out, a, b, c):
        assert t is None or t.is_contiguous()
    check(lib().made_add3(_p(out), dt_of(out), _p(a), dt_of(a), _p(b), _dt(b), _p(c), _dt(c), out.numel(), b_mod, _stream()), "made_add3")
    return out


def gate_rows(x: Tensor, out: Tensor, *, G: Optional[Tensor] = None, gate: int = 0, scale: float = 1.0, drop=None, drop_ld: int = 0,
              drop_col_div: int = 1, row_skip: Optional[Tensor] = None) -> Tensor:
    rows, cols = x.shape
    assert x.stride(1) == 1 and out.stride(1) == 1 and out.shape == x.shape and (G is None or (G.shape == x.shape and G.stride(1) == 1))
    check(lib().made_gate_rows(_p(x), dt_of(x), x.stride(0), _p(G), _dt(G), G.stride(0) if G is not None else 0, gate, scale,
                               _drop_ptr(drop), drop_ld, drop_col_div, _p(out), dt_of(out), out.stride(0), _p(_f32(row_skip, "row_skip")), rows, cols,
                               _stream()), "made_gate_rows")
    return out


def colsum(x: Tensor, out: Tensor) -> None:
    rows, cols = x.shape
    check(lib().made_colsum(_p(x), dt_of(x), x.stride(0), rows, cols, _p(_f32(out, "out")), _stream()), "made_colsum")


def posbn_relu(x: Tensor, weight: Tensor, bias: Tensor, running_mean: Optional[Tensor], running_var: Optional[Tensor], momentum: float,
               batch_stats: bool, save_mean: Tensor, save_rstd: Tensor, out: Tensor, eps: float = 1e-5) -> Tensor:
    B, T, F = x.shape
    assert x.is_contiguous() and out.is_contiguous() and out.shape == x.shape
    check(lib().made_posbn_relu_fwd(_p(x), dt_of(x), F, _p(_f32(weight, "weight")), _p(_f32(bias, "bias")), _p(_f32(running_mean, "running_mean")),
                                    _p(_f32(running_var, "running_var")), float(momentum), float(eps), int(bool(batch_stats)),
                                    _p(_f32(save_mean, "save_mean")), _p(_f32(save_rstd, "save_rstd")), _p(out), dt_of(out), F, B, T, F, _stream()),
          "made_posbn_relu_fwd")
    return out


def posbn_relu_bwd(x: Tensor, y: Tensor, dy: Tensor, weight: Tensor, save_mean: Tensor, save_rstd: Tensor, batch_stats: bool, dx: Tensor,
                   dweight: Optional[Tensor], dbias: Optional[Tensor]) -> Tensor:
    B, T, F = x.shape
    for t in (x, y, dy, dx):
        assert t.is_contiguous() and tuple(t.shape) == (B, T, F)
    check(lib().made_posbn_relu_bwd(_p(x), dt_of(x), F, _p(y), dt_of(y), F, _p(dy), dt_of(dy), F, _p(_f32(weight, "weight")),
                                    _p(_f32(save_mean, "save_mean")), _p(_f32(save_rstd, "save_rstd")), int(bool(batch_stats)),
                                    _p(dx), dt_of(dx), F, _p(_f32(dweight, "dweight")), _p(_f32(dbias, "dbias")), B, T, F, _stream()),
          "made_posbn_relu_bwd")
    return dx


def set_criterion_bwd(logits: Tensor, spans: Tensor, targets: Tensor, pi: Tensor, ti: Tensor, cnt: Tensor, pq: Optional[Tensor],
                      vid_sum: Optional[Tensor], empty_weight: Tensor, fg: int, weights: Tensor, upstream: Optional[Tensor],
                      d_logits: Tensor, d_spans: Tensor, d_pq: Optional[Tensor], d_vid_sum: Optional[Tensor],
                      temperature: float = 0.07, ld_out: int = 2, through_sigmoid: bool = False) -> None:
    nd, B, Q, _ = logits.shape
    G = targets.shape[1]
    Dc = pq.shape[-1] if pq is not None else 0
    check(lib().made_set_criterion_bwd(_p(logits), _p(spans), _p(targets), _p(pi), _p(ti), _p(cnt), _p(pq), _p(vid_sum),
                                       _p(empty_weight), nd, B, Q, G, Dc, fg, temperature, _p(weights), _p(upstream),
                                       _p(d_logits), _p(d_spans), ld_out, int(through_sigmoid), _p(d_pq), _p(d_vid_sum), _stream()),
          "made_set_criterion_bwd")
```

mgsv_amd/trainer.py:

```python
from __future__ import annotations

import math
import os
from typing import Dict, List, Optional, Tuple

import numpy as np
import torch

from . import _lib, dropout as dr, ops, ops_train as tr, tape as _tape
from .config import MadeConfig
from .engine import MadeEngine
from .ops import Seg, round_up

WIDE_SLICES = 8

Tensor = torch.Tensor
XA = "video_guided_to_music_pooling_cross_transformer"


HEAD_PAD = 64


class MadeTrainer(MadeEngine):
    def __init__(self, cfg: MadeConfig, state_dict: Dict[str, object], device="cuda:0", dtype: str = "f32"):
# ... 429 lines not shown
            ws.update({f"e.{l}.src": E(rows, D), f"e.{l}.srcpos": E(rows, D), f"e.{l}.qkv": E(rows, 3 * D), f"e.{l}.att": E(rows, D),
                       f"e.{l}.lse": E(B * H * L, dtype=f32), f"e.{l}.kbits": E(*ops.attention_bits_shape(B, H, L, L), dtype=torch.int32), f"e.{l}.x": E(rows, D), f"e.{l}.s1": E(rows, D), f"e.{l}.h": E(rows, Fd),
                       f"e.{l}.x2": E(rows, D)})
        ws.update(mem=E(rows, D), mempos=E(rows, D))
        if not concat:
            inner, ra, rv = c.ca_heads * c.ca_dim_head, B * Ta, B * Tv
            ws.update(c_nx=E(ra, D), c_nc=E(rv, D), c_q=E(ra, inner), c_kv=E(rv, 2 * inner), c_att=E(ra, inner), c_lse=E(B * c.ca_heads * Ta, dtype=f32),
                      c_ax=E(ra, D), c_nf=E(ra, D), c_z1=E(ra, c.ca_ffn_dim), c_h=E(ra, c.ca_ffn_dim), c_y=E(ra, D),
                      c_g1=E(ra, D), c_g2=E(ra, D), c_g3=E(ra, D), c_gf=E(ra, c.ca_ffn_dim), c_gq=E(ra, inner), c_gkv=E(rv, 2 * inner),
                      c_gatt=E(ra, inner), c_delta=E(B * c.ca_heads * Ta, dtype=f32), c_dseg=E(ra, D), c_dframe=E(rv, D), c_gnc=E(rv, D))
        i32 = torch.int32
        ws.update(rows_v=(E(B * Tv, dtype=i32), E(1, dtype=i32)), rows_a=(E(B * Ta, dtype=i32), E(1, dtype=i32)), rows_f=(E(rows, dtype=i32), E(1, dtype=i32)),
                  order_v=E(B, dtype=i32), order_a=E(B, dtype=i32), order_f=E(B, dtype=i32))
        ws.update(wide_plan=E(_lib.wide_plan_words(B, self._wide_slots()), dtype=i32))
        BQ = B * Q
        stacks = dict(tgt=E(nd + 1, BQ, D), tq=E(nd + 1, BQ, D), qkv=E(nd, BQ, 3 * D), att=E(nd, BQ, D), t_a=E(nd, BQ, D), t1=E(nd, BQ, D),
                      t1q=E(nd, BQ, D), qc=E(nd, BQ, D), pooled=E(nd, BQ, H * D), attc=E(nd, BQ, D), t_b=E(nd, BQ, D), t2=E(nd, BQ, D),
                      h=E(nd, BQ, Fd), t_c=E(nd, BQ, D),
                      **({"n1": E(nd, BQ, D)} if c.detr_pre_norm else {}),
                      g_ffn=E(nd, BQ, D), g_z=E(nd, BQ, Fd), g_ca=E(nd, BQ, D), g_attc=E(nd, BQ, D), g_q=E(nd, B, HQ, D), g_qc=E(nd, BQ, D),
                      g_sa=E(nd, BQ, D), g_qkv=E(nd, BQ, 3 * D), dt1q=E(nd, BQ, D))
        ws["dstack"] = stacks
        ws["s_stack"] = E(nd, BQ, H, dtype=f32)
        ws["ca_lse"] = E(nd, B * HQ, dtype=f32)
        for l in range(nd):
            ws.update({f"d.{l}.{k}": v[l] for k, v in stacks.items() if not k.startswith("g_")})
            ws.update({f"d.{l}.lse": E(B * H * Q, dtype=f32), f"d.{l}.s": ws["s_stack"][l], f"d.{l}.t3": stacks["tgt"][l + 1]})
        if c.contrastive_align_loss:
            Dc = c.contrastive_hdim
            if c.audio_short_cut:
                ws.update(pq_n0=E(nd * B * Q, Dc, dtype=f32), pq_s1=E(nd * B * Q, Dc, dtype=f32), pq_s2=E(nd * B * Q, Dc, dtype=f32),
                          dpq_s=E(nd * B * Q, Dc, dtype=f32), dpq_s2=E(nd * B * Q, Dc, dtype=f32))
            ws.update(dpq=E(nd * B * Q, Dc, dtype=f32), dvid_sum=ws["dclip"][2 * B * D:2 * B * D + B * Dc].view(B, Dc), dpq_raw=E(nd * B * Q, Dc), dpv_raw=E(B * Tv, Dc),
                      dframe_x=E(B * Tv, D))
        self._tws[key] = ws
        return ws

    @torch.no_grad()
    def same_music_exclusion(self, music_ids) -> Optional[Tensor]:
        c = self.cfg
        if music_ids is None or c.vmr_loss != "dual_single_loss_fuse":
            return None
        ids = list(music_ids)
        code = {}
        idx = torch.tensor([code.setdefault(str(i), len(code)) for i in ids])
        ex = (idx[:, None] == idx[None, :]).float()
        ex.fill_diagonal_(0.0)
        return ex.to(self.device)

    def forward_train(self, frame_feats: Tensor, segment_feats: Tensor, frame_masks: Tensor, segment_masks: Tensor,
                      spans_target: Tensor, seed: int = 0, music_ids=None, v_duration: Optional[Tensor] = None) -> Dict[str, Tensor]:
        c, P = self.cfg, self.P
        self._set_products()
        if c.predict_center == 1 and v_duration is None:
            raise ValueError("predict_center=1 needs v_duration (reference model/model_Uni.py:280-282)")
        self.seed = int(seed)
        B, Tv, _ = frame_feats.shape
        Ta = segment_feats.shape[1]
        concat = "concat" in c.mml_fusion
        D, L, Q, nd, H = c.D, (Tv + Ta if concat else Ta), c.num_moment_queries, c.detr_dec_layers, c.detr_nheads
        ws, tw = self._buffers(B, Tv, Ta), self._train_buffers(B, Tv, Ta)
        fm, sm = frame_masks.contiguous(), segment_masks.contiguous()
        pd = float(c.detr_dropout)
        self._shape = (B, Tv, Ta)
        self._inputs = (frame_feats.contiguous(), segment_feats.contiguous(), fm, sm, spans_target.contiguous())

        fus, fus_mask = ws["fus"], ws["fus_mask"]
        self._groups = {}
        cur, side = torch.cuda.current_stream(), self._side_stream()
        side.wait_stream(cur)
        self._rows = {sm.data_ptr(): ops.row_index(sm, out=tw["rows_a"])}
        self._order = {sm.data_ptr(): ops.batch_order(sm, out=tw["order_a"])}
        with torch.cuda.stream(side):
            ops.concat_cols(fm if concat else None, sm, fus_mask)
            self._rows[fm.data_ptr()] = ops.row_index(fm, out=tw["rows_v"])
            self._order[fm.data_ptr()] = ops.batch_order(fm, out=tw["order_v"])
            self._rows[fus_mask.data_ptr()] = ops.row_index(fus_mask, out=tw["rows_f"])
            self._order[fus_mask.data_ptr()] = ops.batch_order(fus_mask, out=tw["order_f"])
            self._wide_plan = (ops.wide_slice_plan(fus_mask, n_slots=self._wide_slots(), max_slices=WIDE_SLICES,
                                                   order=self._order[fus_mask.data_ptr()], out=tw["wide_plan"])
                               if "regression" not in c.mml_localization and self._wide_planned_ok(B, H * Q, D) else None)
            pos = ops.sine_pe(fus_mask, P["dim_t"], out=ws["pos"])
            self._encode_train(self._inputs[0], fm, "video", ws, tw, 0)
        self._encode_train(self._inputs[1], sm, "audio", ws, tw, Tv)
        cur.wait_stream(side)
        rows_f = self._rows[fus_mask.data_ptr()]
        if concat:
            frame, seg = fus[:, :Tv], fus[:, Tv:]
        else:
            frame, seg = ws["frame_buf"], ws["seg_buf"]
            self._ca_fusion_train(ws, tw, frame, seg, fm, sm, B, Tv, Ta)
        self._views = (frame, seg)
        video, music = ws["video"], ws["music"]
        out: Dict[str, Tensor] = dict(video_feats=video, music_feats=music, frame_feats=frame, segment_feats=seg)

        qp = P["query_embed"]
        hd = D // H
        ca_scale = 1.0 / math.sqrt(hd)
        GQ = tw.get("GQ")
        regression = "regression" in c.mml_localization

        def dec_fill_tgt() -> None:
            tgt = tw["d.0.tgt"]
            if c.moment_query_type in ("video", "music", "xpool"):
                if c.moment_query_type == "xpool":
                    cur.wait_stream(side)
                src_vec = video if c.moment_query_type == "video" else (music if c.moment_query_type == "music" else tw["xpool_q"])
                if Q == 1:
                    tr.add3(tgt, src_vec)
                else:
                    tgt.view(B, Q, D).copy_(src_vec[:, None, :].expand(B, Q, D))
            else:
                _tape.zero_(tgt)
            if Q > 1 and not c.detr_pre_norm:
                tr.add3(tw["d.0.tq"], tgt, qp, b_mod=Q * D)

        stage = self._dec_stage_chain()

        def dec_query_side(l: int) -> None:
            p, d = f"detr_transformer.decoder.layers.{l}", f"d.{l}"
            tgt, tq = tw[d + ".tgt"], tw[d + ".tq"]
            qkv = tw[d + ".qkv"]
            Win, bin_ = P[p + ".ca.in.w"], P[p + ".ca.in.b"]
            Wt = P[p + ".ca.in.wt"]
            if c.detr_pre_norm:
                n1 = tw[d + ".n1"]
                qp_rows = qp.expand(B * Q, D) if Q == 1 else qp.repeat(B, 1)
                if Q == 1:
                    Wsa, bsa = P[p + ".sa.in.w"], P[p + ".sa.in.b"]
                    ops.layernorm(tgt, P[p + ".ln1.g"], P[p + ".ln1.b"], out=n1)
                    ops.linear(n1, Wsa[2 * D:], bsa[2 * D:], out=tw[d + ".att"], drop=self._drop(f"dec.{l}" + ".sa_attn", pd), drop_ld=H, drop_col_div=hd)
                else:
                    ops.layernorm_add(tgt, P[p + ".ln1.g"], P[p + ".ln1.b"], qp_rows, n1, tq)
                    ops.linear(n1, P[p + ".sa.in.w"], P[p + ".sa.in.b"], A2=tq, a2_replace=True,
                               segs=[Seg(out=qkv, col_begin=0, use_a2=True), Seg(out=qkv[:, 2 * D:], col_begin=2 * D, ldo=qkv.stride(0))])
                    q3 = qkv.view(B, Q, 3 * D)
                    ops.attention(q3[:, :, :D], q3[:, :, D:2 * D], q3[:, :, 2 * D:], tw[d + ".att"].view(B, Q, D), H, lse=tw[d + ".lse"],
                                  drop=self._drop(f"dec.{l}" + ".sa_attn", pd))
                ta = ops.linear(tw[d + ".att"], P[p + ".sa.out.w"], P[p + ".sa.out.b"], R=tgt, out=tw[d + ".t_a"], drop=self._drop(f"dec.{l}" + ".drop1", pd))
                ops.layernorm_add(ta, P[p + ".ln2.g"], P[p + ".ln2.b"], qp_rows, tw[d + ".t1"], tw[d + ".t1q"])
                qc = ops.linear(tw[d + ".t1q"], Win[:D], bin_[:D], out=tw[d + ".qc"])
            elif stage:
                Wsa, bsa = P[p + ".sa.in.w"], P[p + ".sa.in.b"]
                sa_drop = dict(drop=self._drop(f"dec.{l}" + ".sa_attn", pd), drop_ld=H, drop_col_div=hd)
                if l == 0:
                    ops.dec_stage(tgt, Wsa[2 * D:], bsa[2 * D:], tw[d + ".att"], **sa_drop)
                else:
                    q_ = f"detr_transformer.decoder.layers.{l - 1}"
                    ops.dec_stage(tw[f"d.{l - 1}.t_c"], Wsa[2 * D:], bsa[2 * D:], tw[d + ".att"], ln=(P[q_ + ".ln3.g"], P[q_ + ".ln3.b"]),
                                  x_out=tgt, **sa_drop)
                ta = ops.linear(tw[d + ".att"], P[p + ".sa.out.w"], P[p + ".sa.out.b"], R=tgt, out=tw[d + ".t_a"], drop=self._drop(f"dec.{l}" + ".drop1", pd))
                qc = ops.dec_stage(ta, Win[:D], bin_[:D], tw[d + ".qc"], ln=(P[p + ".ln1.g"], P[p + ".ln1.b"]), add=qp,
                                   x_out=tw[d + ".t1"], a_out=tw[d + ".t1q"])
            else:
                if Q == 1:
                    Wsa, bsa = P[p + ".sa.in.w"], P[p + ".sa.in.b"]
                    ops.linear(tgt, Wsa[2 * D:], bsa[2 * D:], out=tw[d + ".att"], drop=self._drop(f"dec.{l}" + ".sa_attn", pd), drop_ld=H, drop_col_div=hd)
                else:
                    ops.linear(tgt, P[p + ".sa.in.w"], P[p + ".sa.in.b"], A2=tq, a2_replace=True,
                               segs=[Seg(out=qkv, col_begin=0, use_a2=True), Seg(out=qkv[:, 2 * D:], col_begin=2 * D, ldo=qkv.stride(0))])
                    q3 = qkv.view(B, Q, 3 * D)
                    ops.attention(q3[:, :, :D], q3[:, :, D:2 * D], q3[:, :, 2 * D:], tw[d + ".att"].view(B, Q, D), H, lse=tw[d + ".lse"],
                                  drop=self._drop(f"dec.{l}" + ".sa_attn", pd))
                ta = ops.linear(tw[d + ".att"], P[p + ".sa.out.w"], P[p + ".sa.out.b"], R=tgt, out=tw[d + ".t_a"], drop=self._drop(f"dec.{l}" + ".drop1", pd))
                t1 = tw[d + ".t1"]
                ops.layernorm_add(ta, P[p + ".ln1.g"], P[p + ".ln1.b"], qp.expand(B * Q, D) if Q == 1 else qp.repeat(B, 1), t1, tw[d + ".t1q"])
# ... 72 lines not shown
            s1 = ops.layernorm(x, P[p + (".ln2.g" if pre else ".ln1.g")], P[p + (".ln2.b" if pre else ".ln1.b")], out=tw[e + ".s1"], row_skip=fskip)
            h = ops.linear(s1, P[p + ".ff1.w"], P[p + ".ff1.b"], act=ops.ACT_RELU, out=tw[e + ".h"], rows=rows_f,
                           drop=self._drop(f"enc.{l}" + ".ffn_act", pd))
            x2 = ops.linear(h, P[p + ".ff2.w"], P[p + ".ff2.b"], R=x if pre else s1, out=tw[e + ".x2"], rows=rows_f,
                            drop=self._drop(f"enc.{l}" + ".drop2", pd))
            last = l == c.detr_enc_layers - 1
            if pre:
                xin = x2
                if last:
                    ops.layernorm_add(x2, P["enc.norm.g"], P["enc.norm.b"], pos2, tw["mem"], tw["mempos"], row_skip=fskip)
                continue
            nsrc, nsp = (tw["mem"], tw["mempos"]) if last else (tw[f"e.{l + 1}.src"], tw[f"e.{l + 1}.srcpos"])
            ops.layernorm_add(x2, P[p + ".ln2.g"], P[p + ".ln2.b"], pos2, nsrc, nsp, row_skip=fskip)
        memory, mempos = tw["mem"], tw["mempos"]
        out["memory"] = memory.view(B, L, D)

        if regression:
            return self._regression_train(out, ws, tw, memory.view(B, L, D), fus_mask, v_duration, cur, side)

        mem3, mempos3 = memory.view(B, L, D), mempos.view(B, L, D)
        if dec_early is None:
            dec_fill_tgt()
        hs = ws["hs"]
        GQ = tw["GQ"]
        n_split = int(_lib.variant_env("MADE_WIDE_NSPLIT", "0")) or max(1, min(8, 256 // max(B, 1)))
        wplan = self._wide_plan if _lib.variant_env("MADE_WIDE_PLANNED", "1") != "0" else None
        if wplan is not None:
            n_split = WIDE_SLICES
        t3_stack = tw["dstack"]["tgt"][1:]
        for l in range(nd):
            p, d = f"detr_transformer.decoder.layers.{l}", f"d.{l}"
            tgt, tq = tw[d + ".tgt"], tw[d + ".tq"]
            qkv = tw[d + ".qkv"]
            if l == 0 and dec_early is not None:
                cur.wait_event(dec_early)
            else:
                dec_query_side(l)
            Win, bin_ = P[p + ".ca.in.w"], P[p + ".ca.in.b"]
            qprime, t1 = GQ[:, 1, l], tw[d + ".t1"]
            pooled = tw[d + ".pooled"]
            s_out = tw[d + ".s"] if Q == 1 else tw["s_raw"]
            ops.attention_wide(qprime.view(B, H, Q, D), mempos3, mem3, pooled.view(B, Q, H, D).permute(0, 2, 1, 3), scale=ca_scale,
                               key_mask=fus_mask, drop=self._drop(f"dec.{l}" + ".ca_attn", pd), sum_out=s_out,
                               n_split=n_split, part_o=ws["part_o"], part_ml=ws["part_ml"],
                               lse_out=tw["ca_lse"][l] if stage else None, plan=wplan)
            if Q > 1:
                tw[d + ".s"].view(B, Q, H).copy_(s_out.view(B, H, Q).permute(0, 2, 1))
            attc = tw[d + ".attc"]
            if stage:
                ops.linear(pooled[:, :D], Win[2 * D:2 * D + hd], bin_[2 * D:], M=B * Q, N=hd, K=D, batch=H, a_z_stride=D, w_z_stride=hd * D,
                           segs=[Seg(out=attc, ldo=D, out_z_stride=hd)], bias_row_scale=tw[d + ".s"], bias_z_stride=hd)
            else:
                ops.linear(pooled[:, :D], Win[2 * D:2 * D + hd], None, M=B * Q, N=hd, K=D, batch=H, a_z_stride=D, w_z_stride=hd * D,
                           segs=[Seg(out=attc, ldo=D, out_z_stride=hd)])
                tr.head_bias(attc, tw[d + ".s"], bin_[2 * D:], H)
            if c.detr_pre_norm:
                tb = ops.linear(attc, P[p + ".ca.out.w"], P[p + ".ca.out.b"], R=tw[d + ".t_a"], out=tw[d + ".t_b"], drop=self._drop(f"dec.{l}" + ".drop2", pd))
                t2 = ops.layernorm(tb, P[p + ".ln3.g"], P[p + ".ln3.b"], out=tw[d + ".t2"])
                h = ops.linear(t2, P[p + ".ff1.w"], P[p + ".ff1.b"], act=ops.ACT_RELU, out=tw[d + ".h"], drop=self._drop(f"dec.{l}" + ".ffn_act", pd))
                ops.linear(h, P[p + ".ff2.w"], P[p + ".ff2.b"], R=tb, out=tw[d + ".t3"], drop=self._drop(f"dec.{l}" + ".drop3", pd))
                continue
            tb = ops.linear(attc, P[p + ".ca.out.w"], P[p + ".ca.out.b"], R=t1, out=tw[d + ".t_b"], drop=self._drop(f"dec.{l}" + ".drop2", pd))
            if stage:
                h = ops.dec_stage(tb, P[p + ".ff1.w"], P[p + ".ff1.b"], tw[d + ".h"], ln=(P[p + ".ln2.g"], P[p + ".ln2.b"]), x_out=tw[d + ".t2"],
                                  act=ops.ACT_RELU, drop=self._drop(f"dec.{l}" + ".ffn_act", pd))
                t2 = tw[d + ".t2"]
            else:
                t2 = ops.layernorm(tb, P[p + ".ln2.g"], P[p + ".ln2.b"], out=tw[d + ".t2"])
                h = ops.linear(t2, P[p + ".ff1.w"], P[p + ".ff1.b"], act=ops.ACT_RELU, out=tw[d + ".h"], drop=self._drop(f"dec.{l}" + ".ffn_act", pd))
            tcx = ops.linear(h, P[p + ".ff2.w"], P[p + ".ff2.b"], R=t2, out=tw[d + ".t_c"], drop=self._drop(f"dec.{l}" + ".drop3", pd))
            t3 = tw[d + ".t3"]
            if stage:
                if l + 1 == nd:
                    ops.layernorm(tcx, P[p + ".ln3.g"], P[p + ".ln3.b"], out=t3)
            elif l + 1 < nd:
                ops.layernorm_add(tcx, P[p + ".ln3.g"], P[p + ".ln3.b"], qp.expand(B * Q, D) if Q == 1 else qp.repeat(B, 1), t3, tw[f"d.{l + 1}.tq"])
            else:
                ops.layernorm(tcx, P[p + ".ln3.g"], P[p + ".ln3.b"], out=t3)
        ops.layernorm(t3_stack.reshape(nd * B * Q, D), P["dec.norm.g"], P["dec.norm.b"], out=hs.view(nd * B * Q, D))
        out["hs"] = hs.view(nd, B, Q, D)

        hs2 = hs.view(nd * B * Q, D)
        logits, spans = ws["logits"], ws["spans"]
        ops.linear(hs2, P["class_embed.w"], P["class_embed.b"], out=logits.view(-1, 2))
        h1 = ops.linear(hs2, P["span_embed.0.w"], P["span_embed.0.b"], act=ops.ACT_RELU, out=tw["h1"])
        h2 = ops.linear(h1, P["span_embed.1.w"], P["span_embed.1.b"], act=ops.ACT_RELU, out=tw["h2"])
        if c.predict_center == 1:
            ops.linear(h2, P["span_embed.2.w"], P["span_embed.2.b"], act=ops.ACT_SIGMOID, segs=[Seg(out=spans.view(-1, 2), ldo=2)])
            spans[..., 1] = (v_duration.to(self.device, torch.float32) / c.max_m_duration).view(1, B, 1)
        else:
            ops.linear(h2, P["span_embed.2.w"], P["span_embed.2.b"], act=ops.ACT_SIGMOID, out=spans.view(-1, 2))
        out.update(pred_logits=logits[-1], pred_spans=spans[-1], logits_all=logits, spans_all=spans)
        if c.moment_loss:
            last = hs[nd - 1]
            m1 = ops.linear(last, P["moment_embed.0.w"], P["moment_embed.0.b"], act=ops.ACT_RELU)
            m2 = ops.linear(m1, P["moment_embed.1.w"], P["moment_embed.1.b"], act=ops.ACT_RELU)
            m3 = ops.linear(m2, P["moment_embed.2.w"], P["moment_embed.2.b"], out_dtype=torch.float32)
            mf = ops.l2norm_rows(m3)
            if c.audio_short_cut:
                mq = music if Q == 1 else music[:, None, :].expand(B, Q, D).contiguous()
                tr.add3(m3, mf, mq, b_mod=B * Q * D)
                mf = ops.l2norm_rows(m3)
            out["moment_feats"] = mf.view(B, Q, D)
        pq = vid_sum = None
        if c.contrastive_align_loss:
            ops.linear(hs2, P["proj_q.w"], P["proj_q.b"], out=ws["pq_raw"])
            pq = ws["pq"]
            pq2 = pq.view(nd * B * Q, -1)
            if c.audio_short_cut:
                mq = music if Q == 1 else music[:, None, :].expand(B, Q, D).contiguous()
                ops.l2norm_rows(ws["pq_raw"], out_f32=tw["pq_n0"])
                tr.add3(tw["pq_s1"], tw["pq_n0"], mq, b_mod=B * Q * D)
                ops.l2norm_rows(tw["pq_s1"], out_f32=pq2)
                if c.aux_loss and nd > 1:
                    n_aux = (nd - 1) * B * Q
                    tr.add3(tw["pq_s2"][:n_aux], pq2[:n_aux], mq, b_mod=B * Q * D)
                    ops.l2norm_rows(tw["pq_s2"][:n_aux], out_f32=pq2[:n_aux])
            else:
                ops.l2norm_rows(ws["pq_raw"], out_f32=pq2)
            self._frame_rows_linear(frame, P["proj_v.w"], P["proj_v.b"], ws["pv_raw"], B, Tv)
            pv = ws["pv"]
            ops.l2norm_rows(ws["pv_raw"], out_f32=pv.view(B * Tv, pq.shape[-1]))
            vid_sum = ops.masked_mean(pv, None, out=ws["vid_sum"])
            out.update(proj_queries=pq[-1], proj_vid_mem=pv, proj_queries_all=pq)
        tg = self._inputs[4]
        pi, ti, cnt, status, cost = ops.hungarian_match(logits.view(nd * B, Q, 2), spans.view(nd * B, Q, 2), tg, c.foreground_label)
        losses, total = ops.set_criterion(logits, spans, tg, pi, ti, cnt, pq, vid_sum, P["empty_weight"], c.foreground_label, P["crit_weights"])
        self._match = (pi, ti, cnt)
        out.update(matcher_pred_idx=pi.view(nd, B, -1), matcher_tgt_idx=ti.view(nd, B, -1), matcher_count=cnt.view(nd, B),
                   matcher_status=status, criterion_losses=losses, localization_loss=total)
        cur.wait_stream(side)
        return out

    def _opt_stream(self):
        st = getattr(self, "_opt_st", None)
        if st is None:
            st = self._opt_st = torch.cuda.Stream(device=self.device)
        return st

    def _wide_slots(self) -> int:
        if getattr(self, "_wide_slots_n", None) is None:
            self._wide_slots_n = max(8, min(1024, _lib.device_info()[1]))
        return self._wide_slots_n

    def _wide_planned_ok(self, B: int, HQ: int, D: int) -> bool:
        return self.tc == torch.bfloat16 and D in (256, 512) and HQ <= 32 and B <= self._wide_slots()

    def _dec_stage_chain(self) -> bool:
        c = self.cfg
        return (self.tc == torch.bfloat16 and c.num_moment_queries == 1 and c.D in (256, 512) and not c.detr_pre_norm
                and _lib.variant_env("MADE_DEC_STAGE", "1") != "0")

    def _encode_train(self, feats: Tensor, mask: Tensor, which: str, ws, tw, row_off: int) -> None:
        c, P = self.cfg, self.P
        if c.agg_module == "mlp":
            return self._encode_train_mlp(feats, mask, which, ws, tw, row_off)
        B, T, Kin = feats.shape
        D, Hh = c.D, c.SA_temporal_heads
        proj, mod, pe, depth, tag = (("vit_proj", "video_transformer", "pe_video", c.video_transformer_depth, "v") if which == "video"
                                     else ("ast_proj", "audio_transformer", "pe_audio", c.audio_transformer_depth, "a"))
        cls = bool(c.with_cls_token)
        T1 = T + 1 if cls else T
        if P[pe].shape[0] < T1:
            raise ValueError(f"{which} position table holds {P[pe].shape[0]} positions < {T1}")
        nrow = B * T
        mflat = mask.reshape(-1)
        pt = dr.P_TEMPORAL
        name = "video" if which == "video" else "audio"
        act = ops.ACT_QUICKGELU if c.with_act_after_proj else ops.ACT_NONE
        zp = tw[tag + ".zproj"] if c.with_act_after_proj else None
        x = tw[f"{tag}.0.x0"]
        if cls:
            mask1 = tw[tag + ".mask1"]
            mask1[:, 0] = 1.0; mask1[:, 1:] = mask
            self._rows[mask1.data_ptr()] = ops.row_index(mask1, out=tw[tag + ".rows1"])
            self._order[mask1.data_ptr()] = ops.batch_order(mask1, out=tw[tag + ".order1"])
            x3 = x.view(B, T1, D)
            x3[:, 0] = (P["cls_" + name].float() + P[pe][0].float()).to(self.tc)
            lin_out = dict(segs=[Seg(out=x3[:, 1:], ldo=D, rows_per_batch=T, out_batch_stride=T1 * D)])
            pe_rows = P[pe][1:T1]
        else:
            mask1 = mask
            lin_out = dict(out=x, rows=self._rw(mflat))
            pe_rows = P[pe][:T]
        mflat1 = mask1.reshape(-1)
        rws = self._rw(mflat1)
        if self.tc == torch.bfloat16:
            xin = ops.cast_mask_rows(feats.view(nrow, Kin), mflat, tw[tag + ".xin"])
            ops.linear(xin, P[proj + ".w"], P[proj + ".b"], act=act, Zout=zp, R=pe_rows, r_row_mod=T, **lin_out)
        else:
            ops.linear(feats.view(nrow, Kin), P[proj + ".w"], P[proj + ".b"], a_row_mask=mflat, act=act, Zout=zp, R=pe_rows, r_row_mod=T, **lin_out)
        for l in range(depth):
            p, t = f"{mod}.layers.{l}", f"{tag}.{l}"
            x1 = ops.layernorm(x, P[p + ".ln1.g"], P[p + ".ln1.b"], out=tw[t + ".x1"], row_skip=mflat1)
            qkv = ops.linear(x1, P[p + ".in.w"], P[p + ".in.b"], out=tw[t + ".qkv"], rows=rws)
            q3 = qkv.view(B, T1, 3 * D)
            att = tw[t + ".att"]
            ops.attention(q3[:, :, :D], q3[:, :, D:2 * D], q3[:, :, 2 * D:], att.view(B, T1, D), Hh, key_mask=mask1, q_skip_mask=mask1,
                          lse=tw[t + ".lse"], drop=self._drop(f"{name}.{l}.attn", pt), order=self._order[mask1.data_ptr()],
                          keep_bits=tw[t + ".kbits"] if self._bits else None)
            x2 = ops.linear(att, P[p + ".out.w"], P[p + ".out.b"], R=x1, out=tw[t + ".x2"], rows=rws)
            x3_ = ops.layernorm(x2, P[p + ".ln2.g"], P[p + ".ln2.b"], out=tw[t + ".x3"], row_skip=mflat1)
            h = ops.linear(x3_, P[p + ".ff1.w"], P[p + ".ff1.b"], act=ops.ACT_GELU, out=tw[t + ".h"], Zout=tw[t + ".z1"], rows=rws,
                           drop=self._drop(f"{name}.{l}.ffn_act", pt))
            nxt = tw[f"{tag}.{l + 1}.x0"] if l + 1 < depth else tw[tag + ".xlast"]
            x = ops.linear(h, P[p + ".ff2.w"], P[p + ".ff2.b"], R=x3_, out=nxt, rows=rws, drop=self._drop(f"{name}.{l}.ffn_out", pt))
        if "concat" in c.mml_fusion:
            local = ws["fus"][:, row_off:row_off + T]
        else:
            local = ws["frame_buf"] if which == "video" else ws["seg_buf"]
        vec = ws["video"] if which == "video" else ws["music"]
        if cls:
            y3 = ops.linear(x, P[mod + ".final.w"], P[mod + ".final.b"], out_row_mask=mflat1, out=tw[tag + ".y1"]).view(B, T1, D)
            ops.l2norm_rows(y3[:, 0], out_f32=vec)
            local.copy_(y3[:, 1:])
# ... 108 lines not shown
                 defer: Optional[list] = None, later: Optional[list] = None, **kw) -> Optional[Tensor]:
        rows = self._rw(row_mask)
        gw_ = self.G[key + ".w"] if gw is None else gw
        gb_ = self.G.get(key + ".b") if gb is None else gb
        if later is not None:
            later.append(lambda: tr.gemm_tn(dz, x, gw_, accumulate=True, colsum=gb_, row_mask=row_mask if rows is None else None,
                                            row_groups=self._rg(row_mask), rows=rows))
        elif defer is not None and self._groupable(dz, x, gw_):
            defer.append((dz, x, gw_, gb_))
        else:
            tr.gemm_tn(dz, x, gw_, accumulate=True, colsum=gb_,
                       row_mask=row_mask if rows is None else None, row_groups=self._rg(row_mask), rows=rows)
        if dx_out is None:
            return None
        return ops.linear(dz, self.P[key + ".wt"] if wt is None else wt, None, out=dx_out, tile_skip_mask=skip if rows is None else None,
                          rows=rows, **kw)

    def _rg(self, row_mask: Optional[Tensor]) -> Optional[Tensor]:
        return self._groups.get(row_mask.data_ptr()) if row_mask is not None else None

    def _rw(self, mask: Optional[Tensor]):
        return self._rows.get(mask.data_ptr()) if mask is not None else None

    @torch.no_grad()
    def backward(self, g_ret: Optional[Tensor] = None, g_loc: Optional[Tensor] = None, zero_grad: bool = True, grad_sync=None,
                 early_opt=None) -> None:
        self._set_products()
        c, P, G = self.cfg, self.P, self.G
        B, Tv, Ta = self._shape
        ws, tw = self._buffers(B, Tv, Ta), self._train_buffers(B, Tv, Ta)
        feats_v, feats_a, fm, sm, tg = self._inputs
        concat = "concat" in c.mml_fusion
        D, L, Q, nd, ne, H = c.D, (Tv + Ta if concat else Ta), c.num_moment_queries, c.detr_dec_layers, c.detr_enc_layers, c.detr_nheads
        hd, HQ = D // H, H * Q
        pd = float(c.detr_dropout)
        inv_keep = 1.0 / (1.0 - pd) if (self.training_dropout and pd > 0) else 1.0
        fus, fus_mask = ws["fus"], ws["fus_mask"]
        fskip = fus_mask.view(-1)
        qskip = fus_mask
        regression = "regression" in c.mml_localization
        if regression:
            fskip = qskip = None
        rows = B * L
        if zero_grad and not getattr(self, "_grads_zeroed", False):
            _tape.zero_(self.flat_grad)
        self._grads_zeroed = False
        dvideo, dmusic = tw["dvideo"], tw["dmusic"]
        _tape.zero_(tw["dclip"])
        video, music = ws["video"], ws["music"]
        frame, seg_view = self._views
        cur, side = torch.cuda.current_stream(), self._side_stream()
        xq = c.moment_query_type == "xpool" and not regression
        side.wait_stream(cur)
        ret_done = None
        ret_gen = None
        if not xq:
            ret_main = _lib.variant_env("MADE_RET_BWD_MAIN", "0") == "1"
            ret_split = (_lib.variant_env("MADE_RET_SPLIT", "1") != "0" and not ret_main and not regression
                         and _lib.variant_env("MADE_RET_HANDOFF", "") == "" and _lib.variant_env("MADE_RET_HANDOFF_REV", "") == "")
            with torch.cuda.stream(cur if ret_main else side):
                self._ret_main_stream = cur
                try:
                    self._ret_ck(0)
                    if ret_split:
                        ret_gen = self._retrieval_bwd_gen(ws, tw, g_ret, B, Ta, sm)
                        if next(ret_gen, "done") == "done":
                            ret_gen = None
                    else:
                        self._retrieval_bwd(ws, tw, g_ret, B, Ta, sm)
                    on_main = torch.cuda.current_stream() == cur
                finally:
                    self._ret_main_stream = None
                if ret_gen is None:
                    ret_done = torch.cuda.Event()
                    ret_done.record(cur if on_main else side)

        if regression:
            dmem, dtgt0 = self._regression_bwd(ws, tw, g_loc, B, L), None
        else:
            logits, spans = ws["logits"], ws["spans"]
            pi, ti, cnt = self._match
            pq = ws["pq"] if c.contrastive_align_loss else None
            vid_sum = ws["vid_sum"] if c.contrastive_align_loss else None
            tr.set_criterion_bwd(logits, spans, tg, pi, ti, cnt, pq, vid_sum, P["empty_weight"], c.foreground_label, P["crit_weights"], g_loc,
                                 tw["dlog"], tw["dsp"], tw["dpq"] if pq is not None else None, tw["dvid_sum"] if pq is not None else None,
                                 ld_out=HEAD_PAD, through_sigmoid=True)
            hs2 = ws["hs"].view(nd * B * Q, D)
            dhs = tw["dhs"]
            dlog, dsp = tw["dlog"], tw["dsp"]
            if self.tc != torch.float32:
                tr.add3(tw["dlogsp_c"], tw["dlogsp"])
                dlog, dsp = tw["dlog_c"], tw["dsp_c"]
            heads_dw: list = []
            heads_dw.append(lambda: tr.gemm_tn(dlog[:, :2], hs2, G["class_embed.w"], accumulate=True, colsum=G["class_embed.b"]))
            ops.linear(dlog, P["class_embed.wt"], None, out=dhs)
            n_span = 1 if c.predict_center == 1 else 2
            heads_dw.append(lambda: tr.gemm_tn(dsp[:, :n_span], tw["h2"], G["span_embed.2.w"], accumulate=True, colsum=G["span_embed.2.b"]))
            dz2 = ops.linear(dsp, P["span_embed.2.wt"], None, out=tw["hg1"], gate=_lib.GATE_RELU_OUT, G=tw["h2"])
            dz1 = self._lin_bwd(dz2, tw["h1"], "span_embed.1", dx_out=tw["hg2"], gate=_lib.GATE_RELU_OUT, G=tw["h1"], later=heads_dw)
            self._lin_bwd(dz1, hs2, "span_embed.0", dx_out=dhs, R=dhs, later=heads_dw)
            if c.contrastive_align_loss:
                Dc = pq.shape[-1]
                dn = tw["dpq"]
                if c.audio_short_cut:
                    if c.aux_loss and nd > 1:
                        n_aux = (nd - 1) * B * Q
                        ds2 = tw["dpq_s2"][:n_aux]
                        tr.l2norm_bwd(tw["pq_s2"][:n_aux], dn[:n_aux], dx=ds2)
                        dmusic.add_(ds2.view(nd - 1, B, Q, D).sum((0, 2)))
                        dn[:n_aux].copy_(ds2)
                    tr.l2norm_bwd(tw["pq_s1"], dn, dx=tw["dpq_s"])
                    dmusic.add_(tw["dpq_s"].view(nd, B, Q, D).sum((0, 2)))
                    dn = tw["dpq_s"]
                tr.l2norm_bwd(ws["pq_raw"], dn, dx_alt=tw["dpq_raw"])
                self._lin_bwd(tw["dpq_raw"], hs2, "proj_q", dx_out=dhs, R=dhs, later=heads_dw)
                tr.l2norm_bwd(ws["pv_raw"], tw["dvid_sum"], dx_alt=tw["dpv_raw"], dy_rows_per=Tv)
                heads_dw.append(lambda: tr.gemm_tn(tw["dpv_raw"][:Tv], frame[0], G["proj_v.w"], accumulate=True, colsum=G["proj_v.b"], batch=(B, 1),
                                                   a_zs=(Tv * Dc, 0), b_zs=(frame.stride(0), 0), colsum_zs=(0, 0)))
                ops.linear(tw["dpv_raw"], P["proj_v.wt"], None, out=tw["dframe_x"])

            qp = P["query_embed"]
            mem3, mempos3 = tw["mem"].view(B, L, D), tw["mempos"].view(B, L, D)
            Lp = tw["PdS"].shape[-1]
            GQ, PdS = tw["GQ"], tw["PdS"]
            ca_scale = 1.0 / math.sqrt(hd)
            st = tw["dstack"]
            dtgt = None
            stage = self._dec_stage_chain()
            pre = bool(c.detr_pre_norm)
            S_all = tw["dS_S"]
            if not stage:
                ops.linear(GQ[0, 1].reshape(nd * HQ, D), mempos3[0], None, M=nd * HQ, N=L, K=D, batch=B, a_z_stride=GQ.stride(0), w_z_stride=L * D,
                           segs=[Seg(out=S_all, ldo=Lp, rows_per_batch=HQ, out_batch_stride=B * HQ * Lp, out_z_stride=HQ * Lp)])
            n_split_b = int(_lib.variant_env("MADE_WIDE_NSPLIT", "0")) or max(1, min(8, 256 // max(B, 1)))
            wplan = self._wide_plan if HQ <= 8 and _lib.variant_env("MADE_WIDE_PLANNED", "1") != "0" else None
            if wplan is not None:
                n_split_b = WIDE_SLICES
            if stage:
                gN = tw["dgN"]
                tr.layernorm_bwd(tw["dstack"]["tgt"][1:].reshape(nd * B * Q, D), P["dec.norm.g"], dhs, gN, dgamma=G["dec.norm.g"], dbeta=G["dec.norm.b"])
            for l in range(nd - 1, -1, -1):
                p, d = f"detr_transformer.decoder.layers.{l}", f"d.{l}"
                g1, g2, g4 = tw["dg1"], tw["dg2"], tw["dg4"]
                if stage and _lib.variant_env("MADE_CHAIN_BUFS", "1") != "0":
                    ch = tw["dchain"][l]
                    g1a, g1b, g2a, g2b, g2c, dt_out = ch[0], ch[1], ch[2], ch[3], ch[4], ch[5]
                else:
                    g1a = g1b = g1
                    g2a = g2b = g2c = g2
                    dt_out = tw["dtgt"]
                Win, Wt = P[p + ".ca.in.w"], P[p + ".ca.in.wt"]
                g_ffn, g_z, g_ca, g_attc, g_q, g_qc, g_sa, gqkv = (st[k][l] for k in ("g_ffn", "g_z", "g_ca", "g_attc", "g_q", "g_qc", "g_sa", "g_qkv"))
                if stage:
                    tr.dec_stage_bwd(tw[d + ".t_c"], P[p + ".ln3.g"], gN[l * B * Q:(l + 1) * B * Q], P[p + ".ff2.wt"], g_z,
                                     dgamma_a=G[p + ".ln3.g"], dbeta_a=G[p + ".ln3.b"], add=dtgt, dx_out=g2a, a_out=g_ffn,
                                     drop_a=self._drop(f"dec.{l}" + ".drop3", pd), G=tw[d + ".h"], gate_scale=inv_keep)
                elif pre:
                    tr.layernorm_bwd(tw[d + ".t3"], P["dec.norm.g"], dhs[l * B * Q:(l + 1) * B * Q], g1, dgamma=G["dec.norm.g"], dbeta=G["dec.norm.b"], add=dtgt)
                    tr.gate_rows(g1, g_ffn, drop=self._drop(f"dec.{l}" + ".drop3", pd))
                else:
                    tr.layernorm_bwd(tw[d + ".t3"], P["dec.norm.g"], dhs[l * B * Q:(l + 1) * B * Q], g1, dgamma=G["dec.norm.g"], dbeta=G["dec.norm.b"], add=dtgt)
                    tr.layernorm_bwd(tw[d + ".t_c"], P[p + ".ln3.g"], g1, g2, dgamma=G[p + ".ln3.g"], dbeta=G[p + ".ln3.b"],
                                     dx_drop=g_ffn, drop=self._drop(f"dec.{l}" + ".drop3", pd))
                if not stage:
                    ops.linear(g_ffn, P[p + ".ff2.wt"], None, out=g_z, gate=_lib.GATE_RELU_OUT, G=tw[d + ".h"], gate_scale=inv_keep)
                if pre:
                    dn3 = ops.linear(g_z, P[p + ".ff1.wt"], None, out=g4)
                    tr.layernorm_bwd(tw[d + ".t_b"], P[p + ".ln3.g"], dn3, g2, dgamma=G[p + ".ln3.g"], dbeta=G[p + ".ln3.b"], add=g1,
                                     dx_drop=g_ca, drop=self._drop(f"dec.{l}" + ".drop2", pd))
                    dattc = ops.linear(g_ca, P[p + ".ca.out.wt"], None, out=g_attc)
                else:
                    dt2 = ops.linear(g_z, P[p + ".ff1.wt"], None, out=g1a, R=g2a)
                if pre:
                    pass
                elif stage:
                    dattc = tr.dec_stage_bwd(tw[d + ".t_b"], P[p + ".ln2.g"], dt2, P[p + ".ca.out.wt"], g_attc, dgamma_a=G[p + ".ln2.g"],
                                             dbeta_a=G[p + ".ln2.b"], dx_out=g2b, a_out=g_ca, drop_a=self._drop(f"dec.{l}" + ".drop2", pd))
                else:
                    tr.layernorm_bwd(tw[d + ".t_b"], P[p + ".ln2.g"], dt2, g2, dgamma=G[p + ".ln2.g"], dbeta=G[p + ".ln2.b"],
                                     dx_drop=g_ca, drop=self._drop(f"dec.{l}" + ".drop2", pd))
                    dattc = ops.linear(g_ca, P[p + ".ca.out.wt"], None, out=g_attc)
                dpooled = GQ[:, 0, l]
                qprime = GQ[:, 1, l]
                if stage:
                    ops.linear(dattc[:, :hd], Wt[:, 2 * D:2 * D + hd], None, M=B * Q, N=D, K=hd, batch=H, a_z_stride=hd, w_z_stride=hd,
                               segs=[Seg(out=dpooled, ldo=D, rows_per_batch=Q, out_batch_stride=dpooled.stride(0), out_z_stride=Q * D)])
                    tr.attention_wide_bwd(qprime, dpooled, tw[d + ".pooled"].view(B, HQ, D), mempos3, mem3, tw["ca_lse"][l].view(B, HQ),
                                          PdS[:, 0, l], PdS[:, 1, l], g_q, scale=ca_scale, key_mask=fus_mask, ssum=tw[d + ".s"].view(B, HQ),
                                          dattc=dattc, vbias=P[p + ".ca.in.b"][2 * D:], hd=hd, drop=self._drop(f"dec.{l}" + ".ca_attn", pd),
                                          n_split=n_split_b, part_dq=ws["part_o"], plan=wplan)
                else:
                    tr.head_bias_bwd(dattc, tw[d + ".s"], P[p + ".ca.in.b"][2 * D:], G[p + ".ca.in.b"][2 * D:], tw["d_ds"], H)
                    d_ds = tw["d_ds"]
                    if Q > 1:
                        tw["dds_raw"].view(B, H, Q).copy_(d_ds.view(B, Q, H).permute(0, 2, 1))
                        d_ds = tw["dds_raw"]
                    ops.linear(dattc[:, :hd], Wt[:, 2 * D:2 * D + hd], None, M=B * Q, N=D, K=hd, batch=H, a_z_stride=hd, w_z_stride=hd,
                               segs=[Seg(out=dpooled, ldo=D, rows_per_batch=Q, out_batch_stride=dpooled.stride(0), out_z_stride=Q * D)])
                    S, dP = S_all[l], tw["dS_dP"]
                    ops.linear(dpooled[0], mem3[0], None, M=HQ, N=L, K=D, batch=B, a_z_stride=dpooled.stride(0), w_z_stride=L * D,
                               segs=[Seg(out=dP, ldo=Lp, out_z_stride=HQ * Lp)])
                    tr.softmax_bwd(S, dP, fus_mask, HQ, ca_scale, PdS[:, 0, l], PdS[:, 1, l], tw["dSt"], HQ, L, extra=d_ds.view(-1),
# ... 748 lines not shown
```

Measured before the change: 14040 pairs/s.

## Group sibling head linears into one launch and fuse criterion-grad bf16 cast

Adds a grouped linear kernel that runs up to four tiny-M linear problems in a single launch, dispatching each block to the matching tiny or t16 body. It is used for the class, span and proj_q forward heads and for the two head backward dx linears. The criterion backward kernel now also writes bf16 copies of the logit and span gradients, which removes the separate add3 cast. The proj_v forward moves earlier, overlapping the video encode, and the proj_v backward work is deferred into the later weight-grad list. All of this cuts kernel-launch count and serialization in the head section, at the cost of more code paths and a larger kernel-argument struct.

```diff
diff --git a/include/made_hip.h b/include/made_hip.h
--- a/include/made_hip.h
+++ b/include/made_hip.h
@@ -126,6 +126,8 @@
 };
 int made_linear_variant(const MadeLinearArgs* args);
 
+int made_linear_group(const MadeLinearArgs* problems, int32_t n, void* stream);
+
 typedef struct MadeDecStageArgs {
     const void*  Zin; int64_t ldz;
     const float* ln_g; const float* ln_b;
@@ -511,6 +513,14 @@
                            float temperature, const float* weights, const float* upstream,
                            float* d_logits, float* d_spans, int64_t ld_out, int32_t through_sigmoid,
                            float* d_proj_queries, float* d_vid_sum, void* stream);
+int made_set_criterion_bwd_cast(const float* pred_logits, const float* pred_spans, const float* targets,
+                                const int64_t* pred_idx, const int64_t* tgt_idx, const int32_t* count,
+                                const float* proj_queries, const float* vid_sum, const float* empty_weight,
+                                int64_t n_layers, int64_t B, int64_t Q, int64_t G, int64_t Dc, int32_t fg_label,
+                                float temperature, const float* weights, const float* upstream,
+                                float* d_logits, float* d_spans, int64_t ld_out, int32_t through_sigmoid,
+                                float* d_proj_queries, float* d_vid_sum,
+                                void* d_logits_c, void* d_spans_c, int32_t c_dtype, void* stream);
 
 #define MADE_ADAM_MAX_GROUPS 4
 #define MADE_ADAM_NORM_BLOCKS 1024
diff --git a/mgsv_amd/_lib.py b/mgsv_amd/_lib.py
--- a/mgsv_amd/_lib.py
+++ b/mgsv_amd/_lib.py
@@ -261,12 +261,15 @@
     "made_posbn_relu_bwd": (C.c_int, [vp, i32, i64, vp, i32, i64, vp, i32, i64, vp, vp, vp, i32, vp, i32, i64, vp, vp, i64, i64, i64, vp]),
     "made_set_criterion_bwd": (C.c_int, [vp, vp, vp, vp, vp, vp, vp, vp, vp, i64, i64, i64, i64, i64, i32, f32, vp, vp,
                                          vp, vp, i64, i32, vp, vp, vp]),
+    "made_set_criterion_bwd_cast": (C.c_int, [vp, vp, vp, vp, vp, vp, vp, vp, vp, i64, i64, i64, i64, i64, i32, f32, vp, vp,
+                                              vp, vp, i64, i32, vp, vp, vp, vp, i32, vp]),
     "made_adam_step": (C.c_int, [vp, vp, vp, vp, i64, C.POINTER(MadeAdamGroup), i32, f32, f32, f32, i64, f32, vp, vp]),
     "made_adam_step_device": (C.c_int, [vp, vp, vp, vp, i64, C.POINTER(MadeAdamGroup), i32, f32, f32, f32, vp, i32, f32, vp, vp]),
     "made_repack": (C.c_int, [vp, i32, i64, vp]),
     "made_row_groups": (C.c_int, [vp, i64, vp, vp]),
     "made_row_index": (C.c_int, [vp, i64, vp, vp, vp]),
     "made_linear_variant": (C.c_int, [C.POINTER(MadeLinearArgs)]),
+    "made_linear_group": (C.c_int, [C.POINTER(MadeLinearArgs), i32, vp]),
     "made_row_affine": (C.c_int, [vp, i32, i64, vp, vp, i64, i32, vp, i32, i64, i64, i64, vp]),
     "made_gate_rows": (C.c_int, [vp, i32, i64, vp, i32, i64, i32, f32, vp, i64, i64, vp, i32, i64, vp, i64, i64, vp]),
     "made_xpool_fused": (C.c_int, [C.POINTER(MadeXpoolFusedArgs), vp]),
diff --git a/mgsv_amd/csrc/linear.hip b/mgsv_amd/csrc/linear.hip
--- a/mgsv_amd/csrc/linear.hip
+++ b/mgsv_amd/csrc/linear.hip
@@ -1255,21 +1255,17 @@
 constexpr int U_BM = 16, U_BN = 16, U_CT_LD = U_BN + 4;
 
 template <bool TRAIN, int SPW>
-__global__ __launch_bounds__(NTHREADS) void linear_t16_kernel(const MadeLinearArgs a) {
-    __shared__ __attribute__((aligned(16))) float Ct[4 * U_BM * U_CT_LD];
+__device__ __forceinline__ void linear_t16_body(const MadeLinearArgs& a, const int bx, const int bz, float* Ct ) {
     const int tid = threadIdx.x;
     const int lane = tid & 63, wave = __builtin_amdgcn_readfirstlane(tid >> 6);
     const int r16 = lane & 15, kq = lane >> 4;
     const int M = (int)a.M, N = (int)a.N, K = (int)a.K;
     const int n_tiles = (N + U_BN - 1) / U_BN, m_tiles = (M + U_BM - 1) / U_BM;
     int tile_m, tile_n;
-    {
-        const int bx = blockIdx.x;
-        if ((n_tiles & 7) == 0) { const int j = bx >> 3; tile_m = j % m_tiles; tile_n = (j / m_tiles) * 8 + (bx & 7); }
-        else { tile_m = bx % m_tiles; tile_n = bx / m_tiles; }
-    }
+    if ((n_tiles & 7) == 0) { const int j = bx >> 3; tile_m = j % m_tiles; tile_n = (j / m_tiles) * 8 + (bx & 7); }
+    else { tile_m = bx % m_tiles; tile_n = bx / m_tiles; }
     const int m0 = tile_m * U_BM, n0 = tile_n * U_BN;
-    const int64_t z = blockIdx.z;
+    const int64_t z = bz;
     int Mv = M;
     if (a.n_rows) { const int nv = *a.n_rows; Mv = nv < M ? nv : M; }
     if (m0 >= Mv) return;
@@ -1363,6 +1359,12 @@
     store8(outp, seg.out_dtype, out_z + orow + (n - colb), v, nvalid, out_vec);
 }
 
+template <bool TRAIN, int SPW>
+__global__ __launch_bounds__(NTHREADS) void linear_t16_kernel(const MadeLinearArgs a) {
+    __shared__ __attribute__((aligned(16))) float Ct[4 * U_BM * U_CT_LD];
+    linear_t16_body<TRAIN, SPW>(a, blockIdx.x, blockIdx.z, Ct);
+}
+
 template <bool TRAIN>
 static void launch_t16(const MadeLinearArgs& a, hipStream_t st) {
     const int steps = (int)(a.K / 32), spw = (steps + 3) / 4;
@@ -1371,6 +1373,44 @@
     else if (spw <= 2) hipLaunchKernelGGL((linear_t16_kernel<TRAIN, 2>), g, block, 0, st, a);
     else if (spw <= 4) hipLaunchKernelGGL((linear_t16_kernel<TRAIN, 4>), g, block, 0, st, a);
     else hipLaunchKernelGGL((linear_t16_kernel<TRAIN, 8>), g, block, 0, st, a);
+}
+
+constexpr int GROUP_MAX = 4;
+enum { GROUP_TINY = 0, GROUP_TINY_TRAIN = 1, GROUP_T16 = 2, GROUP_T16_TRAIN = 3 };
+struct LinearGroupK {
+    MadeLinearArgs p[GROUP_MAX];
+    int32_t end[GROUP_MAX];
+    int32_t tiles[GROUP_MAX];
+    int32_t kind[GROUP_MAX];
+    int32_t spw[GROUP_MAX];
+    int32_t n;
+};
+
+__global__ __launch_bounds__(NTHREADS) void linear_group_kernel(const LinearGroupK g_by_value) {
+    const LinearGroupK& g = *(const LinearGroupK*)__builtin_amdgcn_kernarg_segment_ptr();
+    __shared__ __attribute__((aligned(16))) float Ct[4 * T_BM * T_CT_LD];
+    static_assert(4 * T_BM * T_CT_LD >= 4 * U_BM * U_CT_LD, "linear_group_kernel: LDS tile");
+    const int b = blockIdx.x;
+    int i = 0;
+#pragma unroll
+    for (int j = 1; j < GROUP_MAX; ++j)
+        if (j < g.n && b >= g.end[j - 1]) i = j;
+    const int local = b - (i > 0 ? g.end[i - 1] : 0);
+    const int bz = local / g.tiles[i], bx = local - bz * g.tiles[i];
+    const MadeLinearArgs& a = g.p[i];
+    switch (g.kind[i] * 8 + (g.kind[i] >= GROUP_T16 ? g.spw[i] : 0)) {
+        case GROUP_TINY * 8: linear_tiny_body<false>(a, bx, bz, Ct); break;
+        case GROUP_TINY_TRAIN * 8: linear_tiny_body<true>(a, bx, bz, Ct); break;
+        case GROUP_T16 * 8 + 1: linear_t16_body<false, 1>(a, bx, bz, Ct); break;
+        case GROUP_T16 * 8 + 2: linear_t16_body<false, 2>(a, bx, bz, Ct); break;
+        case GROUP_T16 * 8 + 4: linear_t16_body<false, 4>(a, bx, bz, Ct); break;
+        case GROUP_T16 * 8 + 8: linear_t16_body<false, 8>(a, bx, bz, Ct); break;
+        case GROUP_T16_TRAIN * 8 + 1: linear_t16_body<true, 1>(a, bx, bz, Ct); break;
+        case GROUP_T16_TRAIN * 8 + 2: linear_t16_body<true, 2>(a, bx, bz, Ct); break;
+        case GROUP_T16_TRAIN * 8 + 4: linear_t16_body<true, 4>(a, bx, bz, Ct); break;
+        case GROUP_T16_TRAIN * 8 + 8: linear_t16_body<true, 8>(a, bx, bz, Ct); break;
+        default: break;
+    }
 }
 
 }
@@ -1613,6 +1653,43 @@
     return made_check_launch("made_linear");
 }
 
+extern "C" int made_linear_group(const MadeLinearArgs* problems, int32_t n, void* stream) {
+    MADE_REQUIRE(problems != nullptr, "made_linear_group: null problems");
+    MADE_REQUIRE(n >= 1 && n <= GROUP_MAX, "made_linear_group: n=%d out of [1,%d]", (int)n, GROUP_MAX);
+    LinearGroupK g;
+    memset(&g, 0, sizeof(g));
+    g.n = n;
+    int64_t total = 0;
+    for (int i = 0; i < n; ++i) {
+        const MadeLinearArgs& a = problems[i];
+        { const int rc = linear_validate(a); if (rc != MADE_OK) return rc; }
+        MADE_UNSUPPORTED(a.M > 0, "made_linear_group: problem %d has no rows", i);
+        const int v = pick_variant(a);
+        MADE_UNSUPPORTED(v == MADE_LINEAR_TINY || v == MADE_LINEAR_TINY16,
+                         "made_linear_group: problem %d (M=%lld N=%lld K=%lld) is served by kernel variant %d, not by the tiny-M kernels",
+                         i, (long long)a.M, (long long)a.N, (long long)a.K, v);
+        const bool train = a.gate != MADE_GATE_NONE || a.Zout != nullptr || a.drop.p > 0.f;
+        int64_t tiles;
+        if (v == MADE_LINEAR_TINY16) {
+            const int steps = (int)(a.K / 32), spw = (steps + 3) / 4;
+            g.kind[i] = train ? GROUP_T16_TRAIN : GROUP_T16;
+            g.spw[i] = spw <= 1 ? 1 : (spw <= 2 ? 2 : (spw <= 4 ? 4 : 8));
+            tiles = ((a.M + U_BM - 1) / U_BM) * ((a.N + U_BN - 1) / U_BN);
+        } else {
+            g.kind[i] = train ? GROUP_TINY_TRAIN : GROUP_TINY;
+            tiles = ((a.M + T_BM - 1) / T_BM) * ((a.N + T_BN - 1) / T_BN);
+        }
+        total += tiles * a.batch;
+        MADE_UNSUPPORTED(total < (1LL << 30), "made_linear_group: too many tiles");
+        g.p[i] = a;
+        g.tiles[i] = (int32_t)tiles;
+        g.end[i] = (int32_t)total;
+    }
+    for (int i = n; i < GROUP_MAX; ++i) { g.end[i] = (int32_t)total; g.tiles[i] = 1; }
+    hipLaunchKernelGGL(linear_group_kernel, dim3((unsigned)total), dim3(NTHREADS), 0, (hipStream_t)stream, g);
+    return made_check_launch("made_linear_group");
+}
+
 extern "C" int made_linear_variant(const MadeLinearArgs* args) {
     return args ? pick_variant(*args) : -1;
 }
diff --git a/mgsv_amd/csrc/matcher.hip b/mgsv_amd/csrc/matcher.hip
--- a/mgsv_amd/csrc/matcher.hip
+++ b/mgsv_amd/csrc/matcher.hip
@@ -268,7 +268,8 @@
                                                                      int B, int Q, int G, int Dc, int fg, float temperature,
                                                                      const float* weights, const float* upstream,
                                                                      float* dlogits, float* dspans, int ldo, int through_sigmoid,
-                                                                     float* dproj_q, float* dvid_sum) {
+                                                                     float* dproj_q, float* dvid_sum,
+                                                                     void* dlogits_c, void* dspans_c, int cdt) {
     __shared__ unsigned char matched[CRIT_MAX_BQ];
     __shared__ float lgt[CRIT_MAX_BQ];
     __shared__ float red[4];
@@ -282,9 +283,13 @@
     const float* sp = spans + (int64_t)l * B * Q * 2;
     float* dlg = dlogits + (int64_t)l * B * Q * ldo;
     float* dsp = dspans + (int64_t)l * B * Q * ldo;
+    const int64_t lc = (int64_t)l * B * Q * ldo;
     for (int i = tid; i < B * Q; i += CRIT_THREADS) {
         matched[i] = 0;
-        if (slice == 0) { dsp[ldo * i] = 0.f; dsp[ldo * i + 1] = 0.f; }
+        if (slice == 0) {
+            dsp[ldo * i] = 0.f; dsp[ldo * i + 1] = 0.f;
+            if (dspans_c) { store_from_f32(dspans_c, cdt, lc + ldo * i, 0.f); store_from_f32(dspans_c, cdt, lc + ldo * i + 1, 0.f); }
+        }
     }
     __syncthreads();
     float npairs = 0.f;
@@ -326,6 +331,7 @@
             if (through_sigmoid) { dc *= pc * (1.f - pc); dw *= pw * (1.f - pw); }
             dsp[(b * Q + q) * ldo] = dc;
             dsp[(b * Q + q) * ldo + 1] = dw;
+            if (dspans_c) { store_from_f32(dspans_c, cdt, lc + (b * Q + q) * ldo, dc); store_from_f32(dspans_c, cdt, lc + (b * Q + q) * ldo + 1, dw); }
         }
     }
     __syncthreads();
@@ -336,8 +342,10 @@
         float e0 = expf(l0 - mx), e1 = expf(l1 - mx);
         float p0 = e0 / (e0 + e1), p1 = e1 / (e0 + e1);
         const float w = up * weights[2] * empty_w[cls] / (float)(B * Q);
-        dlg[i * ldo] = w * (p0 - (cls == 0 ? 1.f : 0.f));
-        dlg[i * ldo + 1] = w * (p1 - (cls == 1 ? 1.f : 0.f));
+        const float d0 = w * (p0 - (cls == 0 ? 1.f : 0.f)), d1 = w * (p1 - (cls == 1 ? 1.f : 0.f));
+        dlg[i * ldo] = d0;
+        dlg[i * ldo + 1] = d1;
+        if (dlogits_c) { store_from_f32(dlogits_c, cdt, lc + i * ldo, d0); store_from_f32(dlogits_c, cdt, lc + i * ldo + 1, d1); }
     }
     if (proj_q && vid_sum && dproj_q && dvid_sum) {
         const int nrow = ((B - slice + nslice - 1) / nslice) * Q;
@@ -415,6 +423,21 @@
                                       float temperature, const float* weights, const float* upstream,
                                       float* d_logits, float* d_spans, int64_t ld_out, int32_t through_sigmoid,
                                       float* d_proj_queries, float* d_vid_sum, void* stream) {
+    return made_set_criterion_bwd_cast(pred_logits, pred_spans, targets, pred_idx, tgt_idx, count, proj_queries, vid_sum, empty_weight, n_layers, B, Q, G,
+                                       Dc, fg_label, temperature, weights, upstream, d_logits, d_spans, ld_out, through_sigmoid, d_proj_queries,
+                                       d_vid_sum, nullptr, nullptr, MADE_F32, stream);
+}
+
+extern "C" int made_set_criterion_bwd_cast(const float* pred_logits, const float* pred_spans, const float* targets,
+                                           const int64_t* pred_idx, const int64_t* tgt_idx, const int32_t* count,
+                                           const float* proj_queries, const float* vid_sum, const float* empty_weight,
+                                           int64_t n_layers, int64_t B, int64_t Q, int64_t G, int64_t Dc, int32_t fg_label,
+                                           float temperature, const float* weights, const float* upstream,
+                                           float* d_logits, float* d_spans, int64_t ld_out, int32_t through_sigmoid,
+                                           float* d_proj_queries, float* d_vid_sum,
+                                           void* d_logits_c, void* d_spans_c, int32_t c_dtype, void* stream) {
+    MADE_REQUIRE((d_logits_c == nullptr) == (d_spans_c == nullptr), "made_set_criterion_bwd: the converted copies come together");
+    MADE_REQUIRE(c_dtype == MADE_F32 || c_dtype == MADE_BF16, "made_set_criterion_bwd: bad c_dtype %d", (int)c_dtype);
     MADE_REQUIRE(pred_logits && pred_spans && targets && pred_idx && tgt_idx && count && empty_weight && weights && d_logits && d_spans,
                  "made_set_criterion_bwd: null pointer");
     MADE_REQUIRE(n_layers >= 1 && B >= 1 && Q >= 1 && G >= 1, "made_set_criterion_bwd: bad dims");
@@ -423,6 +446,6 @@
     hipLaunchKernelGGL(criterion_bwd_kernel, dim3((unsigned)n_layers, nslice), dim3(CRIT_THREADS), 0, (hipStream_t)stream, pred_logits, pred_spans,
                        targets, pred_idx, tgt_idx, count, proj_queries, vid_sum, empty_weight, (int)B, (int)Q, (int)G, (int)Dc,
                        (int)fg_label, temperature, weights, upstream, d_logits, d_spans, (int)(ld_out > 0 ? ld_out : 2), (int)through_sigmoid,
-                       d_proj_queries, d_vid_sum);
+                       d_proj_queries, d_vid_sum, d_logits_c, d_spans_c, (int)c_dtype);
     return made_check_launch("made_set_criterion_bwd");
 }
diff --git a/mgsv_amd/ops.py b/mgsv_amd/ops.py
--- a/mgsv_amd/ops.py
+++ b/mgsv_amd/ops.py
@@ -145,14 +145,14 @@
 LINEAR_LOG = None
 
 
-def linear(A: Tensor, W: Tensor, bias: Optional[Tensor] = None, *, out: Optional[Tensor] = None,
+def _linear_build(A: Tensor, W: Tensor, bias: Optional[Tensor] = None, *, out: Optional[Tensor] = None,
            segs: Optional[Sequence[Seg]] = None, A2: Optional[Tensor] = None, a2_row_mod: int = 0,
            a2_replace: bool = False, a_row_mask: Optional[Tensor] = None, act: int = ACT_NONE, R: Optional[Tensor] = None,
            r_row_mod: int = 0, out_row_mask: Optional[Tensor] = None, out_dtype: Optional[torch.dtype] = None,
            tile_skip_mask: Optional[Tensor] = None, batch: int = 1, a_z_stride: int = 0, w_z_stride: int = 0, M: Optional[int] = None,
            N: Optional[int] = None, K: Optional[int] = None, gate: int = 0, G: Optional[Tensor] = None, gate_scale: float = 1.0,
            Zout: Optional[Tensor] = None, drop=None, drop_ld: Optional[int] = None, rows=None, drop_col_div: int = 1,
-           bias_row_scale: Optional[Tensor] = None, bias_z_stride: int = 0) -> Tensor:
+           bias_row_scale: Optional[Tensor] = None, bias_z_stride: int = 0):
     assert A.dim() == 2 and W.dim() == 2 and A.stride(1) == 1 and W.stride(1) == 1
     M = A.shape[0] if M is None else M
     K = A.shape[1] if K is None else K
@@ -217,9 +217,25 @@
                            f"G={None if G is None else str(G.dtype)[6:]} Z={None if Zout is None else str(Zout.dtype)[6:]} "
                            f"drop={0 if drop is None else drop[2]}/{drop_col_div} rows={int(rows is not None)} orm={int(out_row_mask is not None)} "
                            f"arm={int(a_row_mask is not None)} out={str(segs[0].out.dtype)[6:]} rpb={segs[0].rows_per_batch} tr={int(any(s_.transposed for s_ in segs))}"))
-    _timed(kind, flops, nbytes, lambda: check(lib().made_linear(C.byref(a), _stream()), "made_linear"),
-           ("rows", rows[1], M) if rows is not None else ((desc, tile_skip_mask, 128) if tile_skip_mask is not None else desc))
+    return a, segs, kind, flops, nbytes, ("rows", rows[1], M) if rows is not None else ((desc, tile_skip_mask, 128) if tile_skip_mask is not None else desc)
+
+
+def linear(A: Tensor, W: Tensor, bias: Optional[Tensor] = None, **kw) -> Tensor:
+    a, segs, kind, flops, nbytes, desc = _linear_build(A, W, bias, **kw)
+    _timed(kind, flops, nbytes, lambda: check(lib().made_linear(C.byref(a), _stream()), "made_linear"), desc)
     return segs[0].out
+
+
+def linear_group(problems: Sequence[dict]) -> list:
+    assert 1 <= len(problems) <= 4, "linear_group: 1..4 problems"
+    built = [_linear_build(**p) for p in problems]
+    arr = (MadeLinearArgs * len(built))()
+    for i, b in enumerate(built):
+        C.memmove(C.byref(arr, i * C.sizeof(MadeLinearArgs)), C.byref(b[0]), C.sizeof(MadeLinearArgs))
+    desc = "group[" + " | ".join(str(b[5]) for b in built) + "]"
+    _timed("linear_group_kernel", sum(b[3] for b in built), sum(b[4] for b in built),
+           lambda: check(lib().made_linear_group(arr, len(built), _stream()), "made_linear_group"), desc)
+    return [b[1][0].out for b in built]
 
 
 def row_index(mask: Tensor, out=None):
diff --git a/mgsv_amd/ops_train.py b/mgsv_amd/ops_train.py
--- a/mgsv_amd/ops_train.py
+++ b/mgsv_amd/ops_train.py
@@ -410,10 +410,18 @@
 def set_criterion_bwd(logits: Tensor, spans: Tensor, targets: Tensor, pi: Tensor, ti: Tensor, cnt: Tensor, pq: Optional[Tensor],
                       vid_sum: Optional[Tensor], empty_weight: Tensor, fg: int, weights: Tensor, upstream: Optional[Tensor],
                       d_logits: Tensor, d_spans: Tensor, d_pq: Optional[Tensor], d_vid_sum: Optional[Tensor],
-                      temperature: float = 0.07, ld_out: int = 2, through_sigmoid: bool = False) -> None:
+                      temperature: float = 0.07, ld_out: int = 2, through_sigmoid: bool = False,
+                      d_logits_c: Optional[Tensor] = None, d_spans_c: Optional[Tensor] = None) -> None:
     nd, B, Q, _ = logits.shape
     G = targets.shape[1]
     Dc = pq.shape[-1] if pq is not None else 0
+    if d_logits_c is not None:
+        assert d_spans_c is not None and d_spans_c.dtype == d_logits_c.dtype and d_logits_c.is_contiguous() and d_spans_c.is_contiguous()
+        check(lib().made_set_criterion_bwd_cast(_p(logits), _p(spans), _p(targets), _p(pi), _p(ti), _p(cnt), _p(pq), _p(vid_sum),
+                                                _p(empty_weight), nd, B, Q, G, Dc, fg, temperature, _p(weights), _p(upstream),
+                                                _p(d_logits), _p(d_spans), ld_out, int(through_sigmoid), _p(d_pq), _p(d_vid_sum),
+                                                _p(d_logits_c), _p(d_spans_c), dt_of(d_logits_c), _stream()), "made_set_criterion_bwd_cast")
+        return
     check(lib().made_set_criterion_bwd(_p(logits), _p(spans), _p(targets), _p(pi), _p(ti), _p(cnt), _p(pq), _p(vid_sum),
                                        _p(empty_weight), nd, B, Q, G, Dc, fg, temperature, _p(weights), _p(upstream),
                                        _p(d_logits), _p(d_spans), ld_out, int(through_sigmoid), _p(d_pq), _p(d_vid_sum), _stream()),
diff --git a/mgsv_amd/trainer.py b/mgsv_amd/trainer.py
--- a/mgsv_amd/trainer.py
+++ b/mgsv_amd/trainer.py
@@ -535,6 +535,9 @@
                                if "regression" not in c.mml_localization and self._wide_planned_ok(B, H * Q, D) else None)
             pos = ops.sine_pe(fus_mask, P["dim_t"], out=ws["pos"])
             self._encode_train(self._inputs[0], fm, "video", ws, tw, 0)
+            pv_early = concat and c.contrastive_align_loss and "regression" not in c.mml_localization and self._heads_grouped()
+            if pv_early:
+                self._proj_v_fwd(fus[:, :Tv], ws, B, Tv)
         self._encode_train(self._inputs[1], sm, "audio", ws, tw, Tv)
         cur.wait_stream(side)
         rows_f = self._rows[fus_mask.data_ptr()]
@@ -773,8 +776,17 @@
 
         hs2 = hs.view(nd * B * Q, D)
         logits, spans = ws["logits"], ws["spans"]
-        ops.linear(hs2, P["class_embed.w"], P["class_embed.b"], out=logits.view(-1, 2))
-        h1 = ops.linear(hs2, P["span_embed.0.w"], P["span_embed.0.b"], act=ops.ACT_RELU, out=tw["h1"])
+        grouped = self._heads_grouped()
+        if grouped:
+            sib = [dict(A=hs2, W=P["class_embed.w"], bias=P["class_embed.b"], out=logits.view(-1, 2)),
+                   dict(A=hs2, W=P["span_embed.0.w"], bias=P["span_embed.0.b"], act=ops.ACT_RELU, out=tw["h1"])]
+            if c.contrastive_align_loss:
+                sib.append(dict(A=hs2, W=P["proj_q.w"], bias=P["proj_q.b"], out=ws["pq_raw"]))
+            ops.linear_group(sib)
+            h1 = tw["h1"]
+        else:
+            ops.linear(hs2, P["class_embed.w"], P["class_embed.b"], out=logits.view(-1, 2))
+            h1 = ops.linear(hs2, P["span_embed.0.w"], P["span_embed.0.b"], act=ops.ACT_RELU, out=tw["h1"])
         h2 = ops.linear(h1, P["span_embed.1.w"], P["span_embed.1.b"], act=ops.ACT_RELU, out=tw["h2"])
         if c.predict_center == 1:
             ops.linear(h2, P["span_embed.2.w"], P["span_embed.2.b"], act=ops.ACT_SIGMOID, segs=[Seg(out=spans.view(-1, 2), ldo=2)])
@@ -795,7 +807,8 @@
             out["moment_feats"] = mf.view(B, Q, D)
         pq = vid_sum = None
         if c.contrastive_align_loss:
-            ops.linear(hs2, P["proj_q.w"], P["proj_q.b"], out=ws["pq_raw"])
+            if not grouped:
+                ops.linear(hs2, P["proj_q.w"], P["proj_q.b"], out=ws["pq_raw"])
             pq = ws["pq"]
             pq2 = pq.view(nd * B * Q, -1)
             if c.audio_short_cut:
@@ -809,10 +822,9 @@
                     ops.l2norm_rows(tw["pq_s2"][:n_aux], out_f32=pq2[:n_aux])
             else:
                 ops.l2norm_rows(ws["pq_raw"], out_f32=pq2)
-            self._frame_rows_linear(frame, P["proj_v.w"], P["proj_v.b"], ws["pv_raw"], B, Tv)
-            pv = ws["pv"]
-            ops.l2norm_rows(ws["pv_raw"], out_f32=pv.view(B * Tv, pq.shape[-1]))
-            vid_sum = ops.masked_mean(pv, None, out=ws["vid_sum"])
+            if not pv_early:
+                self._proj_v_fwd(frame, ws, B, Tv)
+            pv, vid_sum = ws["pv"], ws["vid_sum"]
             out.update(proj_queries=pq[-1], proj_vid_mem=pv, proj_queries_all=pq)
         tg = self._inputs[4]
         pi, ti, cnt, status, cost = ops.hungarian_match(logits.view(nd * B, Q, 2), spans.view(nd * B, Q, 2), tg, c.foreground_label)
@@ -822,6 +834,18 @@
                    matcher_status=status, criterion_losses=losses, localization_loss=total)
         cur.wait_stream(side)
         return out
+
+    def _heads_grouped(self) -> bool:
+        c = self.cfg
+        return (self.tc == torch.bfloat16 and c.num_moment_queries == 1 and not c.audio_short_cut and c.predict_center != 1
+                and "regression" not in c.mml_localization and _lib.variant_env("MADE_HEADS_GROUPED", "1") != "0")
+
+    def _proj_v_fwd(self, frame: Tensor, ws, B: int, Tv: int) -> None:
+        P = self.P
+        self._frame_rows_linear(frame, P["proj_v.w"], P["proj_v.b"], ws["pv_raw"], B, Tv)
+        pv = ws["pv"]
+        ops.l2norm_rows(ws["pv_raw"], out_f32=pv.view(B * Tv, pv.shape[-1]))
+        ops.masked_mean(pv, None, out=ws["vid_sum"])
 
     def _opt_stream(self):
         st = getattr(self, "_opt_st", None)
@@ -1096,21 +1120,32 @@
             pi, ti, cnt = self._match
             pq = ws["pq"] if c.contrastive_align_loss else None
             vid_sum = ws["vid_sum"] if c.contrastive_align_loss else None
+            grouped = self._heads_grouped()
             tr.set_criterion_bwd(logits, spans, tg, pi, ti, cnt, pq, vid_sum, P["empty_weight"], c.foreground_label, P["crit_weights"], g_loc,
                                  tw["dlog"], tw["dsp"], tw["dpq"] if pq is not None else None, tw["dvid_sum"] if pq is not None else None,
-                                 ld_out=HEAD_PAD, through_sigmoid=True)
+                                 ld_out=HEAD_PAD, through_sigmoid=True,
+                                 d_logits_c=tw["dlog_c"] if grouped else None, d_spans_c=tw["dsp_c"] if grouped else None)
             hs2 = ws["hs"].view(nd * B * Q, D)
             dhs = tw["dhs"]
             dlog, dsp = tw["dlog"], tw["dsp"]
-            if self.tc != torch.float32:
+            if grouped:
+                dlog, dsp = tw["dlog_c"], tw["dsp_c"]
+            elif self.tc != torch.float32:
                 tr.add3(tw["dlogsp_c"], tw["dlogsp"])
                 dlog, dsp = tw["dlog_c"], tw["dsp_c"]
             heads_dw: list = []
             heads_dw.append(lambda: tr.gemm_tn(dlog[:, :2], hs2, G["class_embed.w"], accumulate=True, colsum=G["class_embed.b"]))
-            ops.linear(dlog, P["class_embed.wt"], None, out=dhs)
             n_span = 1 if c.predict_center == 1 else 2
             heads_dw.append(lambda: tr.gemm_tn(dsp[:, :n_span], tw["h2"], G["span_embed.2.w"], accumulate=True, colsum=G["span_embed.2.b"]))
-            dz2 = ops.linear(dsp, P["span_embed.2.wt"], None, out=tw["hg1"], gate=_lib.GATE_RELU_OUT, G=tw["h2"])
+            if grouped:
+                ops.linear_group([dict(A=dlog, W=P["class_embed.wt"], out=dhs),
+                                  dict(A=dsp, W=P["span_embed.2.wt"], out=tw["hg1"], gate=_lib.GATE_RELU_OUT, G=tw["h2"])])
+                dz2 = tw["hg1"]
+                if c.contrastive_align_loss:
+                    tr.l2norm_bwd(ws["pq_raw"], tw["dpq"], dx_alt=tw["dpq_raw"])
+            else:
+                ops.linear(dlog, P["class_embed.wt"], None, out=dhs)
+                dz2 = ops.linear(dsp, P["span_embed.2.wt"], None, out=tw["hg1"], gate=_lib.GATE_RELU_OUT, G=tw["h2"])
             dz1 = self._lin_bwd(dz2, tw["h1"], "span_embed.1", dx_out=tw["hg2"], gate=_lib.GATE_RELU_OUT, G=tw["h1"], later=heads_dw)
             self._lin_bwd(dz1, hs2, "span_embed.0", dx_out=dhs, R=dhs, later=heads_dw)
             if c.contrastive_align_loss:
@@ -1126,12 +1161,21 @@
                     tr.l2norm_bwd(tw["pq_s1"], dn, dx=tw["dpq_s"])
                     dmusic.add_(tw["dpq_s"].view(nd, B, Q, D).sum((0, 2)))
                     dn = tw["dpq_s"]
-                tr.l2norm_bwd(ws["pq_raw"], dn, dx_alt=tw["dpq_raw"])
+                if not grouped:
+                    tr.l2norm_bwd(ws["pq_raw"], dn, dx_alt=tw["dpq_raw"])
                 self._lin_bwd(tw["dpq_raw"], hs2, "proj_q", dx_out=dhs, R=dhs, later=heads_dw)
-                tr.l2norm_bwd(ws["pv_raw"], tw["dvid_sum"], dx_alt=tw["dpv_raw"], dy_rows_per=Tv)
+                pv_bwd = lambda: tr.l2norm_bwd(ws["pv_raw"], tw["dvid_sum"], dx_alt=tw["dpv_raw"], dy_rows_per=Tv)
+                if grouped:
+                    heads_dw.append(pv_bwd)
+                else:
+                    pv_bwd()
                 heads_dw.append(lambda: tr.gemm_tn(tw["dpv_raw"][:Tv], frame[0], G["proj_v.w"], accumulate=True, colsum=G["proj_v.b"], batch=(B, 1),
                                                    a_zs=(Tv * Dc, 0), b_zs=(frame.stride(0), 0), colsum_zs=(0, 0)))
-                ops.linear(tw["dpv_raw"], P["proj_v.wt"], None, out=tw["dframe_x"])
+                pv_dx = lambda: ops.linear(tw["dpv_raw"], P["proj_v.wt"], None, out=tw["dframe_x"])
+                if grouped:
+                    heads_dw.append(pv_dx)
+                else:
+                    pv_dx()
 
             qp = P["query_embed"]
             mem3, mempos3 = tw["mem"].view(B, L, D), tw["mempos"].view(B, L, D)
```

Measured after the change: 14130 pairs/s, median of 5. About the same (+0.6%).
